# apple/swift-homomorphic-encryption

Hardware: NVIDIA H100
Metric: BFV ct*ct mults/sec at N=8192, 4 coefficient moduli (higher is better)
Workload: dtype u64

## Files before the change

### swift-homomorphic-encryption_b200/csrc/behz.cu

```cuda
#include <cstdlib>

#include "kernels.cuh"

namespace hecuda {

constexpr int kThreads = 128;

static int cols_per_thread() {
    static const int v = [] {
        const char *e = std::getenv("HECUDA_BEHZ_COLS");
        return (e && e[0] == '1') ? 1 : 2;
    }();
    return v;
}

template <int COLS>
struct Cols {
    u64 v[COLS];
};
template <int COLS>
__device__ __forceinline__ Cols<COLS> ldc(const u64 *p) {
    Cols<COLS> r;
    if (COLS == 2) {
        const ulonglong2 t = *reinterpret_cast<const ulonglong2 *>(p);
        r.v[0] = t.x;
        r.v[COLS - 1] = t.y;
    } else {
        r.v[0] = *p;
    }
    return r;
}
template <int COLS>
__device__ __forceinline__ void stc(u64 *p, const u64 (&v)[COLS]) {
    if (COLS == 2) *reinterpret_cast<ulonglong2 *>(p) = make_ulonglong2(v[0], v[COLS - 1]);
    else *p = v[0];
}

template <int L, int COLS>
__global__ void __launch_bounds__(kThreads) lift_kernel(const u64 *__restrict__ in, int polys_in, u64 *__restrict__ ext,
                                                       int ext_polys, int out_poly_offset,
                                                       const __grid_constant__ LiftConsts c, int n, bool q_rows) {
    const int rows_out = q_rows ? 2 * L + 1 : L + 1, aux0 = q_rows ? L : 0;
    const int coeff = (blockIdx.x * kThreads + threadIdx.x) * COLS;
    if (coeff >= n) return;
    const int64_t poly = (int64_t)blockIdx.z * gridDim.y + blockIdx.y;
    const int64_t item = polys_in == 2 ? (poly >> 1) : poly / polys_in;
    const int pin = (int)(poly - item * polys_in);
    const u64 *src = in + poly * L * n + coeff;
    u64 *dst = ext + ((item * ext_polys + out_poly_offset + pin) * rows_out) * n + coeff;
    u64 z[COLS][L];
    u32 acc_mt[COLS];
#pragma unroll
    for (int k = 0; k < COLS; ++k) acc_mt[k] = 0;
#pragma unroll
    for (int i = 0; i < L; ++i) {
        const Cols<COLS> x = ldc<COLS>(src + (int64_t)i * n);
        if (q_rows) stc<COLS>(dst + (int64_t)i * n, x.v);
#pragma unroll
        for (int k = 0; k < COLS; ++k) {
            z[k][i] = shoup_mul(x.v[k], c.in_w[i], c.in_wp[i], c.q[i]);
            acc_mt[k] += (u32)z[k][i] * c.punct_mt[i];
        }
    }
    u32 r[COLS];
    bool neg[COLS];
#pragma unroll
    for (int k = 0; k < COLS; ++k) {
        r[k] = (acc_mt[k] * c.neg_inv_q_mt) & c.mt_mask;
        neg[k] = r[k] >= c.mt_half;
    }
#pragma unroll
    for (int j = 0; j <= L; ++j) {
        u64 o[COLS];
#pragma unroll
        for (int k = 0; k < COLS; ++k) {
            const u64 rc = neg[k] ? (u64)r[k] + c.neg_off[j] : (u64)r[k];
            u128 acc = (u128)rc * c.qr[j];
#pragma unroll
            for (int i = 0; i < L; ++i) mac128(acc, z[k][i], c.mat[j][i]);
            const u64 red = mont_reduce(acc, c.b[j], c.b_ninv[j]);
            o[k] = c.wide_sums ? barrett64(red, c.b[j], c.b_mu1[j]) : csub(red, c.b[j]);
        }
        stc<COLS>(dst + (int64_t)(aux0 + j) * n, o);
    }
}

struct TensorConsts {
    int R;
    u64 p[kMaxRows], ninv[kMaxRows];
};

template <int COLS>
__global__ void __launch_bounds__(kThreads) tensor_kernel(const u64 *__restrict__ ext, u64 *__restrict__ ten,
                                                         const __grid_constant__ TensorConsts c, int n) {
    const int R = c.R;
    const int row = blockIdx.y;
    const int64_t item = blockIdx.z;
    const int coeff = (blockIdx.x * kThreads + threadIdx.x) * COLS;
    if (coeff >= n) return;
    const u64 p = c.p[row], ninv = c.ninv[row];
    const u64 *e = ext + (item * 4 * R + row) * n + coeff;
    const int64_t ps = (int64_t)R * n;
    const Cols<COLS> a0 = ldc<COLS>(e), a1 = ldc<COLS>(e + ps), b0 = ldc<COLS>(e + 2 * ps), b1 = ldc<COLS>(e + 3 * ps);
    u64 *o = ten + (item * 3 * R + row) * n + coeff;
    u64 o0[COLS], o1[COLS], o2[COLS];
#pragma unroll
    for (int k = 0; k < COLS; ++k) {
        o0[k] = csub(mont_reduce((u128)a0.v[k] * b0.v[k], p, ninv), p);
        u128 m = (u128)a0.v[k] * b1.v[k];
        mac128(m, a1.v[k], b0.v[k]);
        o1[k] = csub(mont_reduce(m, p, ninv), p);
        o2[k] = csub(mont_reduce((u128)a1.v[k] * b1.v[k], p, ninv), p);
    }
    stc<COLS>(o, o0);
    stc<COLS>(o + ps, o1);
    stc<COLS>(o + 2 * ps, o2);
}

struct TensorSumConsts {
    int R;
    long long max_pairs;
    u64 p[kMaxRows], ninv[kMaxRows], mu1[kMaxRows], mu_hi[kMaxRows], mu_lo[kMaxRows];
};

__global__ void __launch_bounds__(kThreads) tensor_sum_kernel(const u64 *__restrict__ ext, u64 *__restrict__ ten,
                                                             const __grid_constant__ TensorSumConsts c, int n,
                                                             long long pairs) {
    const int R = c.R;
    const int row = blockIdx.y;
    const int64_t group = blockIdx.z;
    const int coeff = (blockIdx.x * kThreads + threadIdx.x) * 2;
    if (coeff >= n) return;
    const u64 p = c.p[row], ninv = c.ninv[row];
    const int64_t ps = (int64_t)R * n;
    const u64 *e = ext + (group * pairs * 4 * R + row) * n + coeff;
    u128 a0[2] = {0, 0}, a1[2] = {0, 0}, a2[2] = {0, 0};
    long long since = 0;
    for (long long k = 0; k < pairs; ++k, e += 4 * ps) {
        const Cols<2> l0 = ldc<2>(e), l1 = ldc<2>(e + ps), r0 = ldc<2>(e + 2 * ps), r1 = ldc<2>(e + 3 * ps);
#pragma unroll
        for (int j = 0; j < 2; ++j) {
            mac128(a0[j], l0.v[j], r0.v[j]);
            mac128(a1[j], l0.v[j], r1.v[j]);
            mac128(a1[j], l1.v[j], r0.v[j]);
            mac128(a2[j], l1.v[j], r1.v[j]);
        }
        if (++since >= c.max_pairs) {
            since = 0;
#pragma unroll
            for (int j = 0; j < 2; ++j) {
                u128w w0 = {(u64)a0[j], (u64)(a0[j] >> 64)}, w1 = {(u64)a1[j], (u64)(a1[j] >> 64)},
                      w2 = {(u64)a2[j], (u64)(a2[j] >> 64)};
                a0[j] = barrett128(w0, p, c.mu_hi[row], c.mu_lo[row]);
                a1[j] = barrett128(w1, p, c.mu_hi[row], c.mu_lo[row]);
                a2[j] = barrett128(w2, p, c.mu_hi[row], c.mu_lo[row]);
            }
        }
    }
    u64 *o = ten + (group * 3 * R + row) * n + coeff;
    u64 o0[2], o1[2], o2[2];
    const u64 mu1 = c.mu1[row];
#pragma unroll
    for (int j = 0; j < 2; ++j) {
        o0[j] = barrett64(mont_reduce(a0[j], p, ninv), p, mu1);
        o1[j] = barrett64(mont_reduce(a1[j], p, ninv), p, mu1);
        o2[j] = barrett64(mont_reduce(a2[j], p, ninv), p, mu1);
    }
    stc<2>(o, o0);
    stc<2>(o + ps, o1);
    stc<2>(o + 2 * ps, o2);
}

template <int L, int COLS>
__global__ void __launch_bounds__(kThreads) floor_kernel(const u64 *__restrict__ in, u64 *__restrict__ out,
                                                        const __grid_constant__ FloorConsts c, int n) {
    constexpr int R = 2 * L + 1;
    const int coeff = (blockIdx.x * kThreads + threadIdx.x) * COLS;
    if (coeff >= n) return;
    const int64_t poly = (int64_t)blockIdx.z * gridDim.y + blockIdx.y;
    const u64 *src = in + poly * R * n + coeff;
    u64 *dst = out + poly * L * n + coeff;
    u64 y[COLS][L];
#pragma unroll
    for (int i = 0; i < L; ++i) {
        const Cols<COLS> x = ldc<COLS>(src + (int64_t)i * n);
#pragma unroll
        for (int k = 0; k < COLS; ++k) y[k][i] = shoup_mul(x.v[k], c.inq_w[i], c.inq_wp[i], c.q[i]);
    }
    u64 f[COLS][L + 1];
#pragma unroll
    for (int j = 0; j <= L; ++j) {
        const Cols<COLS> xb = ldc<COLS>(src + (int64_t)(L + j) * n);
#pragma unroll
        for (int k = 0; k < COLS; ++k) {
            u128 acc = (u128)xb.v[k] * c.fq[j];
#pragma unroll
            for (int i = 0; i < L; ++i) mac128(acc, y[k][i], c.fmat[j][i]);
            f[k][j] = mont_reduce(acc, c.b[j], c.b_ninv[j]);
        }
    }
    const u64 msk = c.b[L];
    u64 outv[L][COLS];
#pragma unroll
    for (int k = 0; k < COLS; ++k) {
        u64 w[L];
        u128 acc = (u128)f[k][L] * c.a_msk;
#pragma unroll
        for (int i = 0; i < L; ++i) {
            w[i] = shoup_mul(f[k][i], c.inb_w[i], c.inb_wp[i], c.b[i]);
            mac128(acc, w[i], c.amat[i]);
        }
        u64 alpha = mont_reduce(acc, msk, c.b_ninv[L]);
        alpha = c.wide_sums ? barrett64(alpha, msk, c.msk_mu1) : csub(csub(csub(alpha, 4 * msk), 2 * msk), msk);
        const bool exceeds = alpha > (msk >> 1);
        const u64 alpha_c = exceeds ? msk - alpha : alpha;
#pragma unroll
        for (int i = 0; i < L; ++i) {
            u128 o = (u128)alpha_c * (exceeds ? c.b_mod_q[i] : c.neg_b_mod_q[i]);
#pragma unroll
            for (int kk = 0; kk < L; ++kk) mac128(o, w[kk], c.omat[i][kk]);
            outv[i][k] = csub(csub(mont_reduce(o, c.q[i], c.q_ninv[i]), 2 * c.q[i]), c.q[i]);
        }
    }
#pragma unroll
    for (int i = 0; i < L; ++i) stc<COLS>(dst + (int64_t)i * n, outv[i]);
}

__global__ void __launch_bounds__(kThreads) lift_generic_kernel(const u64 *__restrict__ in, int polys_in, u64 *__restrict__ ext,
                                                               int ext_polys, int out_poly_offset,
                                                               const __grid_constant__ LiftConsts c, int n, bool q_rows) {
    const int L = c.L, rows_out = q_rows ? 2 * L + 1 : L + 1, aux0 = q_rows ? L : 0;
    const int coeff = blockIdx.x * kThreads + threadIdx.x;
    if (coeff >= n) return;
    const int64_t poly = (int64_t)blockIdx.z * gridDim.y + blockIdx.y;
    const int64_t item = poly / polys_in;
    const int pin = (int)(poly - item * polys_in);
    const u64 *src = in + poly * L * n + coeff;
    u64 *dst = ext + ((item * ext_polys + out_poly_offset + pin) * rows_out) * n + coeff;
    u64 z[kMaxL];
    u32 acc_mt = 0;
    for (int i = 0; i < L; ++i) {
        const u64 x = src[(int64_t)i * n];
        if (q_rows) dst[(int64_t)i * n] = x;
        z[i] = shoup_mul(x, c.in_w[i], c.in_wp[i], c.q[i]);
        acc_mt += (u32)z[i] * c.punct_mt[i];
    }
    const u32 r = (acc_mt * c.neg_inv_q_mt) & c.mt_mask;
    const bool neg = r >= c.mt_half;
    for (int j = 0; j <= L; ++j) {
        const u64 rc = neg ? (u64)r + c.neg_off[j] : (u64)r;
        u128 acc = (u128)rc * c.qr[j];
        for (int i = 0; i < L; ++i) mac128(acc, z[i], c.mat[j][i]);
        const u64 red = mont_reduce(acc, c.b[j], c.b_ninv[j]);
        dst[(int64_t)(aux0 + j) * n] = c.wide_sums ? barrett64(red, c.b[j], c.b_mu1[j]) : csub(red, c.b[j]);
    }
}

__global__ void __launch_bounds__(kThreads) floor_generic_kernel(const u64 *__restrict__ in, u64 *__restrict__ out,
                                                                const __grid_constant__ FloorConsts c, int n) {
    const int L = c.L, R = 2 * L + 1;
    const int coeff = blockIdx.x * kThreads + threadIdx.x;
    if (coeff >= n) return;
    const int64_t poly = (int64_t)blockIdx.z * gridDim.y + blockIdx.y;
    const u64 *src = in + poly * R * n + coeff;
    u64 *dst = out + poly * L * n + coeff;
    u64 y[kMaxL], f[kMaxL + 1], w[kMaxL];
    for (int i = 0; i < L; ++i) y[i] = shoup_mul(src[(int64_t)i * n], c.inq_w[i], c.inq_wp[i], c.q[i]);
    for (int j = 0; j <= L; ++j) {
        u128 acc = (u128)src[(int64_t)(L + j) * n] * c.fq[j];
        for (int i = 0; i < L; ++i) mac128(acc, y[i], c.fmat[j][i]);
        f[j] = mont_reduce(acc, c.b[j], c.b_ninv[j]);
    }
    const u64 msk = c.b[L];
    u128 acc = (u128)f[L] * c.a_msk;
    for (int i = 0; i < L; ++i) {
        w[i] = shoup_mul(f[i], c.inb_w[i], c.inb_wp[i], c.b[i]);
        mac128(acc, w[i], c.amat[i]);
    }
    u64 alpha = mont_reduce(acc, msk, c.b_ninv[L]);
    alpha = c.wide_sums ? barrett64(alpha, msk, c.msk_mu1) : csub(csub(csub(alpha, 4 * msk), 2 * msk), msk);
    const bool exceeds = alpha > (msk >> 1);
    const u64 alpha_c = exceeds ? msk - alpha : alpha;
    for (int i = 0; i < L; ++i) {
        u128 o = (u128)alpha_c * (exceeds ? c.b_mod_q[i] : c.neg_b_mod_q[i]);
        for (int kk = 0; kk < L; ++kk) mac128(o, w[kk], c.omat[i][kk]);
        dst[(int64_t)i * n] = barrett64(mont_reduce(o, c.q[i], c.q_ninv[i]), c.q[i], c.q_mu1[i]);
    }
}

#define HE_DISPATCH_L(L_, CALL)                                                                                       \
    switch (L_) {                                                                                                     \
        case 1: { constexpr int LL = 1; CALL; } break;                                                                \
        case 2: { constexpr int LL = 2; CALL; } break;                                                                \
        case 3: { constexpr int LL = 3; CALL; } break;                                                                \
        case 4: { constexpr int LL = 4; CALL; } break;                                                                \
        case 5: { constexpr int LL = 5; CALL; } break;                                                                \
        case 6: { constexpr int LL = 6; CALL; } break;                                                                \
        case 7: { constexpr int LL = 7; CALL; } break;                                                                \
        case 8: { constexpr int LL = 8; CALL; } break;                                                                \
        case 9: { constexpr int LL = 9; CALL; } break;                                                                \
        case 10: { constexpr int LL = 10; CALL; } break;                                                              \
        case 11: { constexpr int LL = 11; CALL; } break;                                                              \
        case 12: { constexpr int LL = 12; CALL; } break;                                                              \
        case 13: { constexpr int LL = 13; CALL; } break;                                                              \
        case 14: { constexpr int LL = 14; CALL; } break;                                                              \
        case 15: { constexpr int LL = 15; CALL; } break;                                                              \
        case 16: { constexpr int LL = 16; CALL; } break;                                                              \
        default: return cudaErrorInvalidValue;                                                                        \
    }

static inline dim3 poly_grid(int64_t n, int64_t polys, int cols) {
    const unsigned gx = (unsigned)((n / cols + kThreads - 1) / kThreads);
    const int64_t gy = polys < 32768 ? polys : 32768;
    return dim3(gx ? gx : 1, (unsigned)gy, (unsigned)((polys + gy - 1) / gy));
}

cudaError_t launch_lift(const Context &ctx, const u64 *in, int polys_in, u64 *ext, int ext_polys, int out_poly_offset,
                        int64_t items, cudaStream_t stream, bool reference_base, bool q_rows) {
    const LiftConsts &consts = reference_base ? ctx.lift : ctx.lift_mul;
    int64_t polys = items * polys_in;
    if (polys == 0) return cudaSuccess;
    const int64_t pstride_in = (int64_t)ctx.L * ctx.n;
    while (polys > 0) {
        int64_t slab = polys >= 32768 ? (polys / 32768) * 32768 : polys;
        const int cols = ctx.L > 16 ? 1 : (ctx.n >= 2 ? cols_per_thread() : 1);
        const dim3 grid = poly_grid(ctx.n, slab, cols);
        ++g_kernel_launches;
        if (ctx.L > 16) {
            lift_generic_kernel<<<grid, kThreads, 0, stream>>>(in, polys_in, ext, ext_polys, out_poly_offset, consts, (int)ctx.n, q_rows);
        } else if (cols == 2) {
            HE_DISPATCH_L(ctx.L, (lift_kernel<LL, 2><<<grid, kThreads, 0, stream>>>(in, polys_in, ext, ext_polys,
                                                                                 out_poly_offset, consts, (int)ctx.n, q_rows)));
        } else {
            HE_DISPATCH_L(ctx.L, (lift_kernel<LL, 1><<<grid, kThreads, 0, stream>>>(in, polys_in, ext, ext_polys,
                                                                                 out_poly_offset, consts, (int)ctx.n, q_rows)));
        }
        in += slab * pstride_in;
        ext += (slab / polys_in) * (int64_t)ext_polys * (q_rows ? 2 * ctx.L + 1 : ctx.L + 1) * ctx.n;
        polys -= slab;
    }
    return cudaGetLastError();
}

cudaError_t launch_tensor(const Context &ctx, const u64 *ext, u64 *ten, int64_t items, cudaStream_t stream,
                          bool reference_base) {
    if (items == 0) return cudaSuccess;
    TensorConsts tc;
    tc.R = 2 * ctx.L + 1;
    const NttRowMap map = reference_base ? ctx.map_qbsk() : ctx.map_qaux();
    for (int r = 0; r < tc.R; ++r) {
        tc.p[r] = ctx.slots[map.slot[r]].dev.p;
        tc.ninv[r] = ctx.slots[map.slot[r]].dev.ninv;
    }
    const int cols = ctx.n >= 2 ? cols_per_thread() : 1;
    const unsigned gx = (unsigned)((ctx.n / cols + kThreads - 1) / kThreads);
    for (int64_t done = 0; done < items;) {
        const int64_t chunk = (items - done) > 65535 ? 65535 : (items - done);
        dim3 grid(gx ? gx : 1, (unsigned)tc.R, (unsigned)chunk);
        ++g_kernel_launches;
        if (cols == 2)
            tensor_kernel<2><<<grid, kThreads, 0, stream>>>(ext + done * 4 * tc.R * ctx.n, ten + done * 3 * tc.R * ctx.n, tc,
                                                            (int)ctx.n);
        else
            tensor_kernel<1><<<grid, kThreads, 0, stream>>>(ext + done * 4 * tc.R * ctx.n, ten + done * 3 * tc.R * ctx.n, tc,
                                                            (int)ctx.n);
        done += chunk;
    }
    return cudaGetLastError();
}

cudaError_t launch_tensor_sum(const Context &ctx, const u64 *ext, u64 *ten, int64_t pairs, int64_t groups,
                              cudaStream_t stream, bool reference_base) {
    if (groups == 0) return cudaSuccess;
    if (ctx.n < 2 || pairs < 1) return cudaErrorInvalidValue;
    TensorSumConsts tc;
    tc.R = 2 * ctx.L + 1;
    const NttRowMap map = reference_base ? ctx.map_qbsk() : ctx.map_qaux();
    u64 pmax = 0;
    for (int r = 0; r < tc.R; ++r) {
        const ModSlot &S = ctx.slots[map.slot[r]].dev;
        tc.p[r] = S.p;
        tc.ninv[r] = S.ninv;
        tc.mu1[r] = S.mu1;
        tc.mu_hi[r] = S.mu_hi;
        tc.mu_lo[r] = S.mu_lo;
        pmax = S.p > pmax ? S.p : pmax;
    }
    const u128 per_pair = 2 * (u128)pmax * pmax;
    const u128 cap = (((u128)1) << 127) / per_pair;
    tc.max_pairs = cap < 1 ? 1 : (cap > (u128)0x7fffffffLL ? 0x7fffffffLL : (long long)cap);
    const unsigned gx = (unsigned)((ctx.n / 2 + kThreads - 1) / kThreads);
    for (int64_t done = 0; done < groups;) {
        const int64_t chunk = (groups - done) > 65535 ? 65535 : (groups - done);
        dim3 grid(gx ? gx : 1, (unsigned)tc.R, (unsigned)chunk);
        ++g_kernel_launches;
        tensor_sum_kernel<<<grid, kThreads, 0, stream>>>(ext + done * pairs * 4 * tc.R * ctx.n, ten + done * 3 * tc.R * ctx.n,
                                                         tc, (int)ctx.n, pairs);
        done += chunk;
    }
    return cudaGetLastError();
}

cudaError_t launch_floor(const Context &ctx, const u64 *in, u64 *out, int64_t polys, cudaStream_t stream,
                         bool reference_base) {
    if (polys == 0) return cudaSuccess;
    const FloorConsts &consts = reference_base ? ctx.floor : ctx.floor_mul;
    const int R = 2 * ctx.L + 1;
    while (polys > 0) {
        int64_t slab = polys >= 32768 ? (polys / 32768) * 32768 : polys;
        const int cols = ctx.L > 16 ? 1 : (ctx.n >= 2 ? cols_per_thread() : 1);
        const dim3 grid = poly_grid(ctx.n, slab, cols);
        ++g_kernel_launches;
        if (ctx.L > 16) {
            floor_generic_kernel<<<grid, kThreads, 0, stream>>>(in, out, consts, (int)ctx.n);
        } else if (cols == 2) {
            HE_DISPATCH_L(ctx.L, (floor_kernel<LL, 2><<<grid, kThreads, 0, stream>>>(in, out, consts, (int)ctx.n)));
        } else {
            HE_DISPATCH_L(ctx.L, (floor_kernel<LL, 1><<<grid, kThreads, 0, stream>>>(in, out, consts, (int)ctx.n)));
        }
        in += slab * (int64_t)R * ctx.n;
        out += slab * (int64_t)ctx.L * ctx.n;
        polys -= slab;
    }
    return cudaGetLastError();
}

}
```

### swift-homomorphic-encryption_b200/csrc/context.cu

```cuda
#include "context.hpp"

#include <cuda_runtime.h>

#include <cmath>
#include <cstdlib>
#include <cstring>

#include "hostmath.hpp"
#include "ntt_fast.cuh"

namespace hecuda {
using namespace host;


static void fill_barrett(u64 p, u64 &mu1, u64 &mu_hi, u64 &mu_lo) {
    mu1 = (u64)(((u128)1 << 64) / p);
    u128 mu = (p & (p - 1)) == 0 ? ((u128)1 << (128 - (bit_length(p) - 1))) : (~(u128)0) / p;
    mu_hi = (u64)(mu >> 64);
    mu_lo = (u64)mu;
}

static bool build_slot(HostSlot &hs, u64 p, int64_t n, int logn, u64 t, std::vector<ulonglong2> &tw,
                       std::vector<ulonglong2> &itw, std::string &err) {
    if (!is_prime(p) || (p - 1) % (2 * (u64)n) != 0) {
        err = "invalidNttModulus: " + std::to_string(p) + " is not a prime = 1 mod 2N";
        return false;
    }
    if (p >= (1ull << 62)) {
        err = "invalidModulus: " + std::to_string(p) + " exceeds 2^62 - 1";
        return false;
    }
    ModSlot &d = hs.dev;
    std::memset(&d, 0, sizeof(d));
    d.p = p;
    fill_barrett(p, d.mu1, d.mu_hi, d.mu_lo);
    d.bits = bit_length(p);
    d.s_prod = d.bits - 2;
    d.mu_prod = (u64)(((u128)1 << (d.bits + 62)) / p);
    d.red_shift = d.bits > 12 ? d.bits - 12 : 0;
    d.red_recip = (u32)((((u128)1) << (d.red_shift + 32)) / p);
    const u64 psi = min_primitive_root(2 * (u64)n, p);
    const u64 psi_inv = invmod(psi, p);
    hs.roots.assign(n, 1);
    hs.inv_roots.assign(n, 1);
    u64 pw = 1, ipw = 1;
    for (int64_t i = 0; i < n; ++i) {
        unsigned r = bitrev((unsigned)i, logn);
        hs.roots[r] = pw;
        hs.inv_roots[r] = ipw;
        pw = mulmod(pw, psi, p);
        ipw = mulmod(ipw, psi_inv, p);
    }
    tw.resize(n);
    itw.resize(n);
    for (int64_t i = 0; i < n; ++i) {
        tw[i] = make_ulonglong2(hs.roots[i], shoup_factor(hs.roots[i], p));
        itw[i] = make_ulonglong2(hs.inv_roots[i], shoup_factor(hs.inv_roots[i], p));
    }
    const u64 n_inv = invmod((u64)n % p, p);
    const u64 w1_inv = n > 1 ? hs.inv_roots[1] : 1;
    d.r64 = (u64)(((u128)1 << 64) % p);
    {
        u64 inv = p;
        for (int i = 0; i < 6; ++i) inv *= 2 - p * inv;
        d.ninv = 0 - inv;
    }
    const u64 scalings[3] = {1 % p, mulmod(t % p, d.r64, p), d.r64};
    for (int k = 0; k < 3; ++k) {
        ModSlot::InvScale &sc = d.inv_scale[k];
        sc.c0 = mulmod(n_inv, scalings[k], p);
        sc.c0p = shoup_factor(sc.c0, p);
        sc.c1 = mulmod(sc.c0, w1_inv, p);
        sc.c1p = shoup_factor(sc.c1, p);
    }
    return true;
}

static DivRoundConsts build_divround(const std::vector<u64> &base) {
    DivRoundConsts c;
    std::memset(&c, 0, sizeof(c));
    c.l = (int)base.size();
    c.last = base.back();
    c.half = c.last >> 1;
    for (int i = 0; i + 1 < c.l; ++i) {
        const u64 m = base[i];
        c.m[i] = m;
        c.mu1[i] = (u64)(((u128)1 << 64) / m);
        c.half_mod[i] = c.half % m;
        c.inv_w[i] = invmod(c.last % m, m);
        c.inv_wp[i] = shoup_factor(c.inv_w[i], m);
    }
    return c;
}

Context *Context::create(int64_t n, const u64 *coeff_moduli, int nmod, u64 t, std::string &err, int word_bits) {
    if (word_bits != 64 && word_bits != 32) { err = "invalidEncryptionParameters: word size must be 32 or 64"; return nullptr; }
    for (int i = 0; i < nmod; ++i)
        if (coeff_moduli[i] >> (word_bits - 2)) { err = "invalidModulus: " + std::to_string(coeff_moduli[i]) + " exceeds the maximum of this word size"; return nullptr; }
    if (n < 2 || (n & (n - 1)) || n > (1 << 17)) { err = "invalidDegree: N must be a power of two in [2, 2^17]"; return nullptr; }
    if (n > (1 << fast::kSplitLogN)) { err = "unsupportedHeOperation: polynomial degrees above 2^" + std::to_string(fast::kSplitLogN) + " are not supported by the NTT kernels"; return nullptr; }
    if (nmod < 1) { err = "invalidEncryptionParameters: need at least one coefficient modulus"; return nullptr; }
    if (nmod > kMaxL) { err = "invalidEncryptionParameters: more than " + std::to_string(kMaxL) + " coefficient moduli (EncryptionParameters.swift:148)"; return nullptr; }
    if (t < 2) { err = "invalidEncryptionParameters: plaintext modulus"; return nullptr; }
    for (int i = 0; i < nmod; ++i)
        for (int j = 0; j < i; ++j)
            if (coeff_moduli[i] == coeff_moduli[j]) { err = "coprimeModuli: repeated coefficient modulus"; return nullptr; }

    Context *c = new Context();
    c->n = n;
    c->logn = bit_length((u64)n) - 1;
    c->has_ks = nmod >= 2;
    c->L = c->has_ks ? nmod - 1 : 1;
    c->t = t;
    c->word_bits = word_bits;
    c->mtilde = word_bits == 64 ? (1ull << 32) : (1ull << 16);
    c->gamma = word_bits == 64 ? ((1ull << 62) - 40797) : ((1ull << 30) - 20405);
    const u64 kMTilde = c->mtilde;
    cudaGetDevice(&c->device);
    c->sm_count = 1;
    cudaDeviceGetAttribute(&c->sm_count, cudaDevAttrMultiProcessorCount, c->device);
    const int L = c->L;
    c->q.assign(coeff_moduli, coeff_moduli + L);
    c->q_ks = c->has_ks ? coeff_moduli[L] : 0;
    for (u64 qi : c->q)
        if (t >= qi) { err = "invalidEncryptionParameters: plaintext modulus must be below every coefficient modulus"; delete c; return nullptr; }
    c->bsk = smallest_ntt_primes(word_bits - 3, L + 1, (u64)n);
    if ((int)c->bsk.size() != L + 1) { err = "notEnoughPrimes for Bsk"; delete c; return nullptr; }
    for (u64 b : c->bsk)
        for (int i = 0; i < nmod; ++i)
            if (b == coeff_moduli[i]) { err = "coprimeModuli: coefficient modulus collides with the BEHZ base"; delete c; return nullptr; }

    c->aux = c->bsk;
    {
        const char *env = std::getenv("HECUDA_AUX_BASE");
        const bool want_fast = !(env && std::string(env) == "reference");
        const int widths[2] = {30, 55};
        double log_q = 0;
        for (u64 v : c->q) log_q += std::log2((double)v);
        const double log_n = (double)c->logn, log_t = std::log2((double)t);
        for (int wi = 0; wi < 2 && want_fast && c->aux == c->bsk && word_bits == 64; ++wi) {
            const bool h_primes = fast::kNarrowHEnabled && std::getenv("HECUDA_AUX_H_PRIMES") != nullptr;
            std::vector<u64> cand = (widths[wi] == 55 && h_primes) ? smallest_ntt_primes(55, L + 1 + nmod, 1ull << 31)
                                                                   : smallest_ntt_primes(widths[wi], L + 1 + nmod, (u64)n);
            std::vector<u64> pick;
            for (u64 v : cand) {
                bool used = false;
                for (int i = 0; i < nmod; ++i) used |= coeff_moduli[i] == v;
                if (!used && (int)pick.size() < L + 1) pick.push_back(v);
            }
            double log_aux = 0, log_aux_l = 0;
            for (size_t j = 0; j < pick.size(); ++j) {
                log_aux += std::log2((double)pick[j]);
                if ((int)j < L) log_aux_l += std::log2((double)pick[j]);
            }
            const bool enough = (int)pick.size() == L + 1 && log_aux >= log_q + log_n + 4 &&
                                log_aux_l + std::log2((double)pick.back()) >= log_t + log_n + log_q + 5;
            if (enough) c->aux = pick;
        }
    }
    c->aux_is_reference = c->aux == c->bsk;

    const int nslots = c->aux_is_reference ? 2 * L + 2 : 3 * L + 3;
    c->slots.resize(nslots);
    std::vector<u64> slot_mod(nslots);
    for (int i = 0; i < L; ++i) slot_mod[c->slot_q(i)] = c->q[i];
    for (int j = 0; j <= L; ++j) slot_mod[c->slot_bsk(j)] = c->bsk[j];
    slot_mod[c->slot_ks()] = c->q_ks;
    if (!c->aux_is_reference)
        for (int j = 0; j <= L; ++j) slot_mod[c->slot_aux(j)] = c->aux[j];
    const size_t table_bytes = sizeof(ulonglong2) * (size_t)n;
    const bool fast = c->logn >= fast::kMinLogN && c->logn <= fast::kMaxLogN;
    const bool split = c->logn == fast::kSplitLogN;
    const int half_logn = c->logn - 1;
    const int64_t half_n = n / 2;
    const int threads = (int)((split ? half_n : n) / 16);
    const size_t tr_bytes = (fast || split) ? sizeof(ulonglong2) * (size_t)15 * threads : 0;
    const size_t half_bytes = sizeof(ulonglong2) * (size_t)half_n;
    const size_t slot_bytes = 2 * table_bytes + (split ? 2 * (2 * half_bytes + 2 * tr_bytes) : 2 * tr_bytes);
    if (cudaMalloc(&c->d_pool, slot_bytes * nslots) != cudaSuccess) { err = "cudaMalloc failed for twiddle tables"; delete c; return nullptr; }
    std::vector<ulonglong2> tw, itw, tr(15 * (size_t)threads), itr(15 * (size_t)threads), twh, itwh;
    std::vector<ModSlot> dev_slots(split ? 3 * nslots : nslots);
    c->split_slot_base = split ? nslots : 0;
    for (int s = 0; s < nslots; ++s) {
        if (s == c->slot_ks() && !c->has_ks) {
            std::memset(&c->slots[s].dev, 0, sizeof(ModSlot));
            dev_slots[s] = c->slots[s].dev;
            continue;
        }
        if (!build_slot(c->slots[s], slot_mod[s], n, c->logn, t, tw, itw, err)) { delete c; return nullptr; }
        char *base = (char *)c->d_pool + slot_bytes * s;
        cudaMemcpy(base, tw.data(), table_bytes, cudaMemcpyHostToDevice);
        cudaMemcpy(base + table_bytes, itw.data(), table_bytes, cudaMemcpyHostToDevice);
        c->slots[s].dev.tw = (const ulonglong2 *)base;
        c->slots[s].dev.itw = (const ulonglong2 *)(base + table_bytes);
        if (fast) {
            for (int k = 0; k < 15; ++k)
                for (int tau = 0; tau < threads; ++tau) {
                    tr[(size_t)k * threads + tau] = tw[fast::fwd_last_source(c->logn, k, tau)];
                    itr[(size_t)k * threads + tau] = itw[fast::inv_first_source(c->logn, k, tau)];
                }
            cudaMemcpy(base + 2 * table_bytes, tr.data(), tr_bytes, cudaMemcpyHostToDevice);
            cudaMemcpy(base + 2 * table_bytes + tr_bytes, itr.data(), tr_bytes, cudaMemcpyHostToDevice);
            c->slots[s].dev.tw_t = (const ulonglong2 *)(base + 2 * table_bytes);
            c->slots[s].dev.itw_t = (const ulonglong2 *)(base + 2 * table_bytes + tr_bytes);
        }
        dev_slots[s] = c->slots[s].dev;
        if (split) {
            for (int hh = 0; hh < 2; ++hh) {
                twh.assign(half_n, tw[0]);
                itwh.assign(half_n, itw[0]);
                for (int64_t i = 1; i < half_n; ++i) {
                    const int sp = bit_length((u64)i) - 1;
                    const int64_t src = ((int64_t)(2 + hh) << sp) + (i - ((int64_t)1 << sp));
                    twh[i] = tw[src];
                    itwh[i] = itw[src];
                }
                for (int k = 0; k < 15; ++k)
                    for (int tau = 0; tau < threads; ++tau) {
                        tr[(size_t)k * threads + tau] = twh[fast::fwd_last_source(half_logn, k, tau)];
                        itr[(size_t)k * threads + tau] = itwh[fast::inv_first_source(half_logn, k, tau)];
                    }
                char *hb = base + 2 * table_bytes + hh * (2 * half_bytes + 2 * tr_bytes);
                cudaMemcpy(hb, twh.data(), half_bytes, cudaMemcpyHostToDevice);
                cudaMemcpy(hb + half_bytes, itwh.data(), half_bytes, cudaMemcpyHostToDevice);
                cudaMemcpy(hb + 2 * half_bytes, tr.data(), tr_bytes, cudaMemcpyHostToDevice);
                cudaMemcpy(hb + 2 * half_bytes + tr_bytes, itr.data(), tr_bytes, cudaMemcpyHostToDevice);
                ModSlot v = c->slots[s].dev;
                v.tw = (const ulonglong2 *)hb;
                v.itw = (const ulonglong2 *)(hb + half_bytes);
                v.tw_t = (const ulonglong2 *)(hb + 2 * half_bytes);
                v.itw_t = (const ulonglong2 *)(hb + 2 * half_bytes + tr_bytes);
                dev_slots[nslots + 2 * s + hh] = v;
            }
        }
    }
    if (cudaMalloc(&c->d_slots, sizeof(ModSlot) * dev_slots.size()) != cudaSuccess) { err = "cudaMalloc failed"; delete c; return nullptr; }
    cudaMemcpy(c->d_slots, dev_slots.data(), sizeof(ModSlot) * dev_slots.size(), cudaMemcpyHostToDevice);

    const u64 *Q = c->q.data();
    auto build_behz = [&](const std::vector<u64> &base, bool reference_base, LiftConsts &lf, FloorConsts &fl) {
    const u64 *BSK = base.data();
    const u64 msk = base[L];
    auto slot_of = [&](int j) { return reference_base ? c->slot_bsk(j) : c->slot_aux(j); };
    std::memset(&lf, 0, sizeof(lf));
    lf.L = L;
    {
        const u64 q_mod_mt = prod_mod(Q, L, kMTilde);
        lf.neg_inv_q_mt = (u32)((kMTilde - invmod(q_mod_mt, kMTilde)) % kMTilde);
    }
    for (int i = 0; i < L; ++i) {
        const u64 qi = Q[i];
        lf.q[i] = qi;
        const u64 inv_punct = invmod(punctured_mod(Q, L, i, qi), qi);
        lf.in_w[i] = mulmod(kMTilde % qi, inv_punct, qi);
        lf.in_wp[i] = shoup_factor(lf.in_w[i], qi);
        lf.punct_mt[i] = (u32)punctured_mod(Q, L, i, kMTilde);
    }
    lf.mt_mask = (u32)(kMTilde - 1);
    lf.mt_half = (u32)(kMTilde >> 1);
    for (int j = 0; j <= L; ++j) lf.neg_off[j] = ((kMTilde + BSK[j] - 1) / BSK[j]) * BSK[j] - kMTilde;
    for (int j = 0; j <= L; ++j) {
        const u64 bj = BSK[j];
        lf.b[j] = bj;
        lf.b_ninv[j] = c->slots[slot_of(j)].dev.ninv;
        const u64 r64 = c->slots[slot_of(j)].dev.r64;
        const u64 mt_inv = mulmod(invmod(kMTilde % bj, bj), r64, bj);
        for (int i = 0; i < L; ++i) lf.mat[j][i] = mulmod(punctured_mod(Q, L, i, bj), mt_inv, bj);
        lf.qr[j] = mulmod(prod_mod(Q, L, bj), mt_inv, bj);
    }
    std::memset(&fl, 0, sizeof(fl));
    fl.L = L;
    const u64 b_mod_msk = prod_mod(BSK, L, msk);
    const u64 r64_msk = c->slots[slot_of(L)].dev.r64;
    const u64 b_inv_msk = mulmod(invmod(b_mod_msk, msk), r64_msk, msk);
    fl.a_msk = (msk - b_inv_msk) % msk;
    for (int i = 0; i < L; ++i) {
        const u64 qi = Q[i];
        fl.q[i] = qi;
        fl.q_ninv[i] = c->slots[c->slot_q(i)].dev.ninv;
        fl.q_mu1[i] = c->slots[c->slot_q(i)].dev.mu1;
        const u64 r64 = c->slots[c->slot_q(i)].dev.r64;
        fl.inq_w[i] = invmod(punctured_mod(Q, L, i, qi), qi);
        fl.inq_wp[i] = shoup_factor(fl.inq_w[i], qi);
        for (int k = 0; k < L; ++k) fl.omat[i][k] = mulmod(punctured_mod(BSK, L, k, qi), r64, qi);
        fl.b_mod_q[i] = mulmod(prod_mod(BSK, L, qi), r64, qi);
        fl.neg_b_mod_q[i] = (qi - fl.b_mod_q[i]) % qi;
    }
    for (int j = 0; j <= L; ++j) {
        const u64 bj = BSK[j];
        fl.b[j] = bj;
        fl.b_ninv[j] = c->slots[slot_of(j)].dev.ninv;
        const u64 q_inv = mulmod(invmod(prod_mod(Q, L, bj), bj), c->slots[slot_of(j)].dev.r64, bj);
        fl.fq[j] = q_inv;
        for (int i = 0; i < L; ++i) {
            const u64 v = mulmod(punctured_mod(Q, L, i, bj), q_inv, bj);
            fl.fmat[j][i] = (bj - v) % bj;
        }
    }
    for (int k = 0; k < L; ++k) {
        const u64 bk = BSK[k];
        fl.inb_w[k] = invmod(punctured_mod(BSK, L, k, bk), bk);
        fl.inb_wp[k] = shoup_factor(fl.inb_w[k], bk);
        fl.amat[k] = mulmod(punctured_mod(BSK, L, k, msk), b_inv_msk, msk);
    }
    };
    build_behz(c->bsk, true, c->lift, c->floor);
    if (c->aux_is_reference) {
        c->lift_mul = c->lift;
        c->floor_mul = c->floor;
    } else {
        build_behz(c->aux, false, c->lift_mul, c->floor_mul);
    }

    auto check_ranges = [&](const std::vector<u64> &base, LiftConsts &lf, FloorConsts &fl) -> bool {
        u64 qmax = 0, bmax = 0;
        for (u64 v : c->q) qmax = v > qmax ? v : qmax;
        for (u64 v : base) bmax = v > bmax ? v : bmax;
        const double worst = std::log2((double)(L + 2)) + std::log2((double)qmax) + std::log2((double)bmax);
        if (worst >= 127.0) return false;
        const bool wide = (u128)bmax + (u128)L * qmax >= ((u128)1 << 64);
        lf.wide_sums = fl.wide_sums = wide ? 1 : 0;
        for (int j = 0; j <= L; ++j) lf.b_mu1[j] = (u64)(((u128)1 << 64) / base[j]);
        fl.msk_mu1 = (u64)(((u128)1 << 64) / base[L]);
        return true;
    };
    if (!check_ranges(c->bsk, c->lift, c->floor) || !check_ranges(c->aux, c->lift_mul, c->floor_mul)) {
        err = "unsupportedHeOperation: " + std::to_string(L) + " ciphertext moduli of this size overflow the 128-bit lazy sums";
        delete c;
        return nullptr;
    }

    {
        u64 mmax = c->q_ks;
        for (u64 v : c->q) mmax = v > mmax ? v : mmax;
        if (std::log2((double)L) + 2 * std::log2((double)mmax) >= 128.0) {
            err = "unsupportedHeOperation: " + std::to_string(L) + " moduli of this size overflow the key-switching accumulator";
            delete c;
            return nullptr;
        }
    }

    c->ks_divround.resize(L + 1);
    c->ms_divround.resize(L + 1);
    for (int l = 1; l <= L; ++l) {
        std::vector<u64> base(c->q.begin(), c->q.begin() + l);
        if (l >= 2) c->ms_divround[l] = build_divround(base);
        if (!c->has_ks) continue;
        base.push_back(c->q_ks);
        c->ks_divround[l] = build_divround(base);
    }
    cudaError_t e = cudaDeviceSynchronize();
    if (e != cudaSuccess) { err = std::string("CUDA error during context setup: ") + cudaGetErrorString(e); delete c; return nullptr; }
    return c;
}

Context::~Context() {
    if (d_pool) cudaFree(d_pool);
    if (d_slots) cudaFree(d_slots);
}

NttRowMap Context::map_q(int rows) const {
    NttRowMap m;
    std::memset(&m, 0, sizeof(m));
    m.rows_per_poly = rows;
    m.group = 1;
    m.src_mod = 0;
    m.src_poly_stride = 0;
    for (int r = 0; r < rows; ++r) m.slot[r] = (unsigned char)slot_q(r);
    return m;
}
NttRowMap Context::map_qbsk() const {
    NttRowMap m;
    std::memset(&m, 0, sizeof(m));
    m.rows_per_poly = 2 * L + 1;
    m.group = 1;
    m.src_mod = 0;
    m.src_poly_stride = 0;
    for (int r = 0; r < L; ++r) m.slot[r] = (unsigned char)slot_q(r);
    for (int j = 0; j <= L; ++j) m.slot[L + j] = (unsigned char)slot_bsk(j);
    return m;
}
NttRowMap Context::map_qaux() const {
    NttRowMap m = map_qbsk();
    if (!aux_is_reference)
        for (int j = 0; j <= L; ++j) m.slot[L + j] = (unsigned char)slot_aux(j);
    return m;
}
NttRowMap Context::map_ks(int l) const {
    NttRowMap m;
    std::memset(&m, 0, sizeof(m));
    m.rows_per_poly = l + 1;
    m.group = 1;
    m.src_mod = 0;
    m.src_poly_stride = 0;
    for (int r = 0; r < l; ++r) m.slot[r] = (unsigned char)slot_q(r);
    m.slot[l] = (unsigned char)slot_ks();
    return m;
}
NttRowMap Context::map_single(int slot) const {
    NttRowMap m;
    std::memset(&m, 0, sizeof(m));
    m.rows_per_poly = 1;
    m.group = 1;
    m.src_mod = 0;
    m.src_poly_stride = 0;
    m.slot[0] = (unsigned char)slot;
    return m;
}
NttRowMap Context::map_ks_digits(int l, long long target_poly_stride) const {
    NttRowMap m = map_ks(l);
    m.rows_per_poly = (l + 1) * l;
    m.group = l;
    m.src_mod = l;
    m.src_poly_stride = target_poly_stride;
    for (int j = 0; j < l; ++j) m.src_slot[j] = (unsigned char)slot_q(j);
    return m;
}
int Context::find_slot(u64 modulus) const {
    for (size_t s = 0; s < slots.size(); ++s)
        if (slots[s].dev.p == modulus) return (int)s;
    return -1;
}

}
```

### swift-homomorphic-encryption_b200/csrc/context.hpp

```cpp
#pragma once
#include <cstdint>
#include <string>
#include <vector>

#include "modarith.cuh"

namespace hecuda {

constexpr int kMaxL = 32;
constexpr int kMaxSlots = 3 * kMaxL + 3;
constexpr int kMaxRows = 2 * kMaxL + 1;

struct ModSlot {
    u64 p;
    u64 mu1;
    u64 mu_hi, mu_lo;
    u64 mu_prod;
    int s_prod;
    int bits;
    int red_shift;
    u32 red_recip;
    u64 ninv;
    u64 r64;
    struct InvScale { u64 c0, c0p, c1, c1p; } inv_scale[3];
    const ulonglong2 *tw;
    const ulonglong2 *itw;
    const ulonglong2 *tw_t;
    const ulonglong2 *itw_t;
};

enum { kScalePlain = 0, kScaleTMont = 1, kScaleMont = 2 };

struct NttRowMap {
    int rows_per_poly;
    int group;
    unsigned char slot[kMaxRows + 1];
    int src_mod;
    long long src_poly_stride;
    unsigned char src_slot[kMaxRows + 1];
};

struct LiftConsts {
    int L;
    int wide_sums;
    u64 b_mu1[kMaxL + 1];
    u64 q[kMaxL];
    u64 in_w[kMaxL], in_wp[kMaxL];
    u32 punct_mt[kMaxL];
    u32 neg_inv_q_mt;
    u32 mt_mask, mt_half;
    u64 neg_off[kMaxL + 1];
    u64 b[kMaxL + 1], b_ninv[kMaxL + 1];
    u64 mat[kMaxL + 1][kMaxL];
    u64 qr[kMaxL + 1];
};

struct FloorConsts {
    int L;
    int wide_sums;
    u64 msk_mu1;
    u64 q[kMaxL], q_ninv[kMaxL], q_mu1[kMaxL];
    u64 inq_w[kMaxL], inq_wp[kMaxL];
    u64 b[kMaxL + 1], b_ninv[kMaxL + 1];
    u64 fq[kMaxL + 1];
    u64 fmat[kMaxL + 1][kMaxL];
    u64 inb_w[kMaxL], inb_wp[kMaxL];
    u64 amat[kMaxL];
    u64 a_msk;
    u64 omat[kMaxL][kMaxL];
    u64 b_mod_q[kMaxL], neg_b_mod_q[kMaxL];
};

struct DivRoundConsts {
    int l;
    u64 m[kMaxL + 1], mu1[kMaxL + 1];
    u64 last, half;
    u64 half_mod[kMaxL + 1];
    u64 inv_w[kMaxL + 1], inv_wp[kMaxL + 1];
};

struct HostSlot {
    ModSlot dev;
    std::vector<u64> roots, inv_roots;
};

class Context {
   public:
    static Context *create(int64_t n, const u64 *coeff_moduli, int nmod, u64 t, std::string &err, int word_bits = 64);
    ~Context();

    int64_t n;
    int logn;
    int word_bits = 64;
    u64 mtilde = 1ull << 32;
    u64 gamma = (1ull << 62) - 40797;
    int L;
    u64 t;
    int device;
    int sm_count;
    std::vector<u64> q;
    u64 q_ks;
    bool has_ks = true;
    std::vector<u64> bsk;
    std::vector<u64> aux;
    bool aux_is_reference = true;
    std::vector<HostSlot> slots;
    ModSlot *d_slots = nullptr;
    int split_slot_base = 0;
    LiftConsts lift;
    FloorConsts floor;
    LiftConsts lift_mul;
    FloorConsts floor_mul;
    std::vector<DivRoundConsts> ks_divround;
    std::vector<DivRoundConsts> ms_divround;
    void *d_pool = nullptr;

    int slot_q(int i) const { return i; }
    int slot_bsk(int j) const { return L + j; }
    int slot_ks() const { return 2 * L + 1; }
    int slot_aux(int j) const { return aux_is_reference ? slot_bsk(j) : 2 * L + 2 + j; }
    NttRowMap map_q(int rows) const;
    NttRowMap map_qbsk() const;
    NttRowMap map_qaux() const;
    NttRowMap map_ks(int l) const;
    NttRowMap map_single(int slot) const;
    NttRowMap map_ks_digits(int l, long long target_poly_stride) const;
    int find_slot(u64 modulus) const;
};

}
```

### swift-homomorphic-encryption_b200/csrc/modarith.cuh

```cuda
#pragma once
#include <cstdint>

#if defined(__CUDACC__)
#define HE_HD __host__ __device__ __forceinline__
#define HE_D __device__ __forceinline__
#else
#define HE_HD inline
#define HE_D inline
#endif

namespace hecuda {

typedef unsigned long long u64;
typedef unsigned int u32;

HE_HD u64 mulhi64(u64 a, u64 b) {
#if defined(__CUDA_ARCH__)
    return __umul64hi(a, b);
#else
    return (u64)(((unsigned __int128)a * b) >> 64);
#endif
}

HE_HD u64 csub(u64 x, u64 p) { return x >= p ? x - p : x; }
HE_HD u64 add_mod(u64 a, u64 b, u64 p) { return csub(a + b, p); }
HE_HD u64 sub_mod(u64 a, u64 b, u64 p) { return csub(a + p - b, p); }

HE_HD u64 shoup_lazy(u64 x, u64 w, u64 wp, u64 p) {
    u64 q = mulhi64(x, wp);
    return x * w - q * p;
}
HE_HD u64 shoup_mul(u64 x, u64 w, u64 wp, u64 p) { return csub(shoup_lazy(x, w, wp, p), p); }

HE_HD u64 barrett64(u64 x, u64 p, u64 mu1) {
    u64 q = mulhi64(x, mu1);
    return csub(x - q * p, p);
}

struct u128w {
    u64 lo, hi;
};
HE_HD u128w mul_wide(u64 a, u64 b) {
    u128w r;
    r.lo = a * b;
    r.hi = mulhi64(a, b);
    return r;
}
HE_HD void mac_wide(u128w &acc, u64 a, u64 b) {
    u64 lo = a * b;
    u64 hi = mulhi64(a, b);
    acc.lo += lo;
    acc.hi += hi + (acc.lo < lo ? 1ull : 0ull);
}

HE_HD u64 barrett128(u128w x, u64 p, u64 mu_hi, u64 mu_lo) {
    u64 ll_hi = mulhi64(x.lo, mu_lo);
    u64 lh_lo = x.lo * mu_hi, lh_hi = mulhi64(x.lo, mu_hi);
    u64 hl_lo = x.hi * mu_lo, hl_hi = mulhi64(x.hi, mu_lo);
    u64 hh_lo = x.hi * mu_hi;
    u64 mid = ll_hi + lh_lo;
    u64 c1 = mid < ll_hi ? 1ull : 0ull;
    u64 mid2 = mid + hl_lo;
    u64 c2 = mid2 < mid ? 1ull : 0ull;
    u64 q = hh_lo + lh_hi + hl_hi + c1 + c2;
    return csub(x.lo - q * p, p);
}

typedef unsigned __int128 u128;
HE_HD void mac128(u128 &acc, u64 a, u64 b) { acc += (u128)a * b; }
HE_HD u64 mont_reduce(u128 acc, u64 p, u64 ninv) {
    const u64 lo = (u64)acc, hi = (u64)(acc >> 64);
    const u64 m = lo * ninv;
    return hi + mulhi64(m, p) + (lo != 0 ? 1ull : 0ull);
}

HE_HD u64 barrett_prod(u128w x, u64 p, u64 mu, int s) {
    u64 xs = (x.lo >> s) | (x.hi << (64 - s));
    u64 q = mulhi64(xs, mu);
    u64 r = x.lo - q * p;
    r = csub(r, 4 * p);
    r = csub(r, 2 * p);
    return csub(r, p);
}

}
```

### swift-homomorphic-encryption_b200/csrc/ntt_fast.cu

```cuda
#include <cuda.h>

#include <mutex>

#include <algorithm>
#include <cstdlib>
#include "kernels.cuh"
#include "ntt_fast.cuh"

namespace hecuda {
using namespace fast;

constexpr int kMaxRowList = 2 * (kMaxL + 1) * kMaxL;
struct RowList {
    int rows_per_poly;
    int count;
    unsigned short row[kMaxRowList];
    unsigned short slot[kMaxRowList];
    unsigned char flags[kMaxRowList];
    unsigned short src_row[kMaxRowList];
    long long src_poly_stride;
};

__device__ __forceinline__ u32 smem_u32(const void *p) { return (u32)__cvta_generic_to_shared(p); }
__device__ __forceinline__ void mbar_init(u64 *bar, int count) {
    asm volatile("mbarrier.init.shared::cta.b64 [%0], %1;" ::"r"(smem_u32(bar)), "r"(count) : "memory");
    asm volatile("fence.mbarrier_init.release.cluster;" ::: "memory");
}
__device__ __forceinline__ void mbar_arrive_expect_tx(u64 *bar, u32 bytes) {
    asm volatile("mbarrier.arrive.expect_tx.shared::cta.b64 _, [%0], %1;" ::"r"(smem_u32(bar)), "r"(bytes) : "memory");
}
__device__ __forceinline__ void mbar_wait(u64 *bar, u32 parity) {
    asm volatile(
        "{\n\t.reg .pred done;\n\t"
        "WAIT_%=:\n\t"
        "mbarrier.try_wait.parity.shared::cta.b64 done, [%0], %1;\n\t"
        "@!done bra WAIT_%=;\n\t}" ::"r"(smem_u32(bar)),
        "r"(parity)
        : "memory");
}
__device__ __forceinline__ void tma_load_1d(void *smem_dst, const void *gmem_src, u32 bytes, u64 *bar) {
    asm volatile("cp.async.bulk.shared::cluster.global.mbarrier::complete_tx::bytes [%0], [%1], %2, [%3];" ::"r"(smem_u32(smem_dst)),
                 "l"(gmem_src), "r"(bytes), "r"(smem_u32(bar))
                 : "memory");
}
__device__ __forceinline__ void tma_load_box(void *smem_dst, const CUtensorMap *map, int line, u64 *bar) {
    asm volatile("cp.async.bulk.tensor.2d.shared::cluster.global.tile.mbarrier::complete_tx::bytes [%0], [%1, {%2, %3}], [%4];" ::"r"(
                     smem_u32(smem_dst)),
                 "l"(map), "r"(0), "r"(line), "r"(smem_u32(bar))
                 : "memory");
}
__device__ __forceinline__ void tma_store_box(const CUtensorMap *map, int line, const void *smem_src) {
    asm volatile("cp.async.bulk.tensor.2d.global.shared::cta.tile.bulk_group [%0, {%1, %2}], [%3];" ::"l"(map), "r"(0), "r"(line),
                 "r"(smem_u32(smem_src))
                 : "memory");
}
__device__ __forceinline__ void tma_prefetch_box(const CUtensorMap *map, int line) {
    asm volatile("cp.async.bulk.prefetch.tensor.2d.L2.global.tile [%0, {%1, %2}];" ::"l"(map), "r"(0), "r"(line) : "memory");
}
__device__ __forceinline__ void tma_commit() { asm volatile("cp.async.bulk.commit_group;" ::: "memory"); }
template <int PENDING>
__device__ __forceinline__ void tma_store_wait_read() { asm volatile("cp.async.bulk.wait_group.read %0;" ::"n"(PENDING) : "memory"); }
__device__ __forceinline__ void tma_store_wait_all() { asm volatile("cp.async.bulk.wait_group 0;" ::: "memory"); }
__device__ __forceinline__ void fence_proxy_async_smem() { asm volatile("fence.proxy.async.shared::cta;" ::: "memory"); }

template <int LOGN, int CLS, int K>
__device__ __forceinline__ void fwd_row_pass(u64 (&x)[16], u64 *sm, int tau, const RowMod &m, bool reduce_in) {
    constexpr int P = plan_passes(LOGN), C = fwd_c(LOGN, K), LB = fwd_lb(LOGN, K);
    load_smem<LOGN, LB, C>(x, sm, tau);
    if (K == 0 && reduce_in) {
#pragma unroll
        for (int r = 0; r < 16; ++r) x[r] = barrett64(x[r], 0 - m.np, m.slot->mu1);
    }
    fwd_pass<LOGN, LB, C, CLS>(x, tau, m);
    if (K == P - 1) fwd_finish<CLS>(x, m);
    store_smem<LOGN, LB, C>(x, sm, tau);
}
template <int LOGN, int CLS>
__device__ __forceinline__ void fwd_row(u64 *sm, int tau, const RowMod &m, bool reduce_in) {
    constexpr int P = plan_passes(LOGN);
    u64 x[16];
    fwd_row_pass<LOGN, CLS, 0>(x, sm, tau, m, reduce_in);
    __syncthreads();
    fwd_row_pass<LOGN, CLS, 1>(x, sm, tau, m, false);
    __syncthreads();
    if (P == 4) {
        fwd_row_pass<LOGN, CLS, (P == 4 ? 2 : 1)>(x, sm, tau, m, false);
        __syncthreads();
    }
    fwd_row_pass<LOGN, CLS, P - 1>(x, sm, tau, m, false);
}

template <int LOGN, int CLS, int K>
__device__ __forceinline__ void inv_row_pass(u64 (&x)[16], u64 *sm, int tau, const RowMod &m) {
    constexpr int C = inv_c(LOGN, K), LB = inv_lb(LOGN, K);
    load_smem<LOGN, LB, C>(x, sm, tau);
    if (narrow_like(CLS) && K > 0 && inv_reduce_at(LOGN, K)) inv_reduce(x, m);
    inv_pass<LOGN, LB, C, CLS, inv_bound_in(LOGN, K)>(x, tau, m);
    if (K == plan_passes(LOGN) - 1 && m.partial) {
        if (CLS == kSmall) {
#pragma unroll
            for (int r = 0; r < 16; ++r) x[r] = csub32((u32)x[r], (u32)(0 - m.np));
        } else {
            reduce_small16(x, m);
        }
    }
    store_smem<LOGN, LB, C>(x, sm, tau);
}
template <int LOGN, int CLS>
__device__ __forceinline__ void inv_row(u64 *sm, int tau, const RowMod &m) {
    constexpr int P = plan_passes(LOGN);
    u64 x[16];
    inv_row_pass<LOGN, CLS, 0>(x, sm, tau, m);
    __syncthreads();
    inv_row_pass<LOGN, CLS, 1>(x, sm, tau, m);
    __syncthreads();
    if (P == 4) {
        inv_row_pass<LOGN, CLS, (P == 4 ? 2 : 1)>(x, sm, tau, m);
        __syncthreads();
    }
    inv_row_pass<LOGN, CLS, P - 1>(x, sm, tau, m);
}

HE_HD constexpr int ntt_row_buffers(int logn) { return logn == 13 ? 2 : 1; }

template <int LOGN>
constexpr size_t ntt_smem_bytes() {
    constexpr int B = ntt_row_buffers(LOGN);
    return sizeof(u64) * B * ((size_t)1 << LOGN) + sizeof(ulonglong2) * ((size_t)1 << (LOGN - 4)) + sizeof(u64) * (B + 1);
}

constexpr int ntt_min_ctas(int logn) { return logn == 13 ? 1 : 1024 / ((1 << logn) / 16); }

template <int LOGN, bool INVERSE>
__global__ void __launch_bounds__((1 << LOGN) / 16, ntt_min_ctas(LOGN))
    ntt_rows_kernel(const __grid_constant__ CUtensorMap map_in, const __grid_constant__ CUtensorMap map_out,
                    const ModSlot *__restrict__ slots, const __grid_constant__ RowList rl, const int polys,
                    const int scale_mode, const int debug_flags) {
    extern __shared__ __align__(1024) u64 smem[];
    constexpr int kLines = (1 << LOGN) / kLineWords;
    constexpr int kBoxes = kLines > kBoxLines ? kLines / kBoxLines : 1;
    constexpr int kLinesPerBox = kLines / kBoxes;
    constexpr u32 kRowBytes = (u32)sizeof(u64) << LOGN, kTwBytes = (u32)sizeof(ulonglong2) << (LOGN - 4);
    constexpr int B = ntt_row_buffers(LOGN), AHEAD = B > 1 ? 1 : 0;
    ulonglong2 *tw_cache = reinterpret_cast<ulonglong2 *>(smem + B * (1 << LOGN));
    u64 *bar_row = reinterpret_cast<u64 *>(tw_cache + (1 << (LOGN - 4)));
    u64 *bar_tw = bar_row + B;
    const int tau = threadIdx.x;
    const int tasks = polys * rl.count;
    auto in_line = [&](int t) {
        const int w = t / polys, p = t - w * polys;
        const int64_t word = INVERSE ? ((int64_t)p * rl.rows_per_poly + rl.row[w]) << LOGN
                                     : (int64_t)p * rl.src_poly_stride + ((int64_t)rl.src_row[w] << LOGN);
        return (int)(word >> 4);
    };
    auto load_row = [&](int t, int buf) {
        mbar_arrive_expect_tx(&bar_row[buf], kRowBytes);
        const int line = in_line(t);
        u64 *dst = smem + buf * (1 << LOGN);
#pragma unroll
        for (int b = 0; b < kBoxes; ++b) tma_load_box(dst + b * kLinesPerBox * kLineWords, &map_in, line + b * kLinesPerBox, &bar_row[buf]);
    };
    if (tau == 0) {
        if (smem_u32(smem) & 1023) __trap();
#pragma unroll
        for (int b = 0; b < B; ++b) mbar_init(&bar_row[b], 1);
        mbar_init(bar_tw, 1);
        if (AHEAD && (int)blockIdx.x < tasks) load_row(blockIdx.x, 0);
    }
    __syncthreads();
    u32 phase_row = 0, phase_tw = 0;
    int cached_slot = -1;
    int buf = 0;
    for (int task = blockIdx.x; task < tasks; task += gridDim.x) {
        const int which = task / polys;
        const int poly = task - which * polys;
        const int flags = rl.flags[which];
        const int slot = rl.slot[which];
        const ModSlot &S = slots[slot];
        u64 *sm = smem + buf * (1 << LOGN);
        const int64_t out_word = ((int64_t)poly * rl.rows_per_poly + rl.row[which]) << LOGN;
        const bool new_slot = slot != cached_slot;
        cached_slot = slot;
        if (tau == 0) {
            if (new_slot) {
                mbar_arrive_expect_tx(bar_tw, kTwBytes);
                tma_load_1d(tw_cache, INVERSE ? S.itw : S.tw, kTwBytes, bar_tw);
            }
            const int fill = task + AHEAD * gridDim.x;
            if (fill < tasks) {
                tma_store_wait_read<B - 1 - AHEAD>();
                load_row(fill, (buf + AHEAD) % B);
            }
            const int next = fill + gridDim.x;
            if (next < tasks && !(debug_flags & 1)) {
                const int line = in_line(next);
#pragma unroll
                for (int b = 0; b < kBoxes; ++b) tma_prefetch_box(&map_in, line + b * kLinesPerBox);
            }
        }
        const int cls = flags & 7;
        RowMod m;
        m.np = 0 - S.p;
        m.kp = (cls == kWide || cls == kSmall) ? 2 * S.p : 4 * S.p;
        m.tw = nullptr;
        m.tw_s = smem_u32(tw_cache);
        m.slot = &S;
        m.scale_mode = INVERSE ? scale_mode : -1;
        m.partial = INVERSE && (flags & 16) != 0;
        if (new_slot) {
            mbar_wait(bar_tw, phase_tw);
            phase_tw ^= 1;
        }
        mbar_wait(&bar_row[buf], (phase_row >> buf) & 1);
        phase_row ^= 1u << buf;
        if (debug_flags & 4) {
        } else
#ifndef HE_EXPERIMENT_ONLY_CLASS
        if (INVERSE) {
            if (kNarrowHEnabled && cls == kNarrowH) inv_row<LOGN, kNarrowHEnabled ? kNarrowH : kNarrow>(sm, tau, m);
            else if (cls == kNarrow) inv_row<LOGN, kNarrow>(sm, tau, m);
            else if (cls == kSmall) inv_row<LOGN, kSmall>(sm, tau, m);
            else if (cls == kMid) inv_row<LOGN, kMid>(sm, tau, m);
            else inv_row<LOGN, kWide>(sm, tau, m);
        } else {
            const bool reduce_in = (flags & 8) != 0;
            if (kNarrowHEnabled && cls == kNarrowH) fwd_row<LOGN, kNarrowHEnabled ? kNarrowH : kNarrow>(sm, tau, m, reduce_in);
            else if (cls == kNarrow) fwd_row<LOGN, kNarrow>(sm, tau, m, reduce_in);
            else if (cls == kSmall) fwd_row<LOGN, kSmall>(sm, tau, m, reduce_in);
            else if (cls == kMid) fwd_row<LOGN, kMid>(sm, tau, m, reduce_in);
            else fwd_row<LOGN, kWide>(sm, tau, m, reduce_in);
        }
#else
        if (INVERSE) inv_row<LOGN, HE_EXPERIMENT_ONLY_CLASS>(sm, tau, m);
        else fwd_row<LOGN, HE_EXPERIMENT_ONLY_CLASS>(sm, tau, m, (flags & 8) != 0);
#endif
        fence_proxy_async_smem();
        __syncthreads();
        if (tau == 0 && !(debug_flags & 2)) {
            const int line = (int)(out_word >> 4);
#pragma unroll
            for (int b = 0; b < kBoxes; ++b) tma_store_box(&map_out, line + b * kLinesPerBox, sm + b * kLinesPerBox * kLineWords);
            tma_commit();
        }
        buf = buf + 1 == B ? 0 : buf + 1;
    }
    if (tau == 0) tma_store_wait_all();
}

__device__ __forceinline__ u32 cluster_ctarank() {
    u32 r;
    asm("mov.u32 %0, %%cluster_ctarank;" : "=r"(r));
    return r;
}
__device__ __forceinline__ int cluster_id_x() {
    u32 r;
    asm("mov.u32 %0, %%clusterid.x;" : "=r"(r));
    return (int)r;
}
__device__ __forceinline__ int cluster_count_x() {
    u32 r;
    asm("mov.u32 %0, %%nclusterid.x;" : "=r"(r));
    return (int)r;
}
__device__ __forceinline__ void cluster_arrive() { asm volatile("barrier.cluster.arrive.release.aligned;" ::: "memory"); }
__device__ __forceinline__ void cluster_wait() { asm volatile("barrier.cluster.wait.acquire.aligned;" ::: "memory"); }
__device__ __forceinline__ void cluster_arrive_relaxed() { asm volatile("barrier.cluster.arrive.relaxed.aligned;" ::: "memory"); }
__device__ __forceinline__ u32 cluster_map(u32 addr, u32 rank) {
    u32 r;
    asm volatile("mapa.shared::cluster.u32 %0, %1, %2;" : "=r"(r) : "r"(addr), "r"(rank));
    return r;
}
__device__ __forceinline__ ulonglong2 ld_cluster_v2(u32 addr) {
    ulonglong2 v;
    asm volatile("ld.shared::cluster.v2.u64 {%0, %1}, [%2];" : "=l"(v.x), "=l"(v.y) : "r"(addr) : "memory");
    return v;
}
__device__ __forceinline__ u64 mont_product(u64 a, u64 b, u64 p, u64 ninv) { return csub(mont_reduce((u128)a * b, p, ninv), p); }

template <int LOGN>
constexpr size_t ntt_tensor_smem_bytes() {
    return sizeof(u64) * 2 * ((size_t)1 << LOGN) + sizeof(ulonglong2) * ((size_t)1 << (LOGN - 4)) + sizeof(u64) * 3;
}

template <int LOGN>
__global__ void __launch_bounds__((1 << LOGN) / 16, 1)
    ntt_forward_tensor_kernel(const __grid_constant__ CUtensorMap map_lhs, const __grid_constant__ CUtensorMap map_rhs,
                              const __grid_constant__ CUtensorMap map_ext, u64 *__restrict__ ten,
                              const ModSlot *__restrict__ slots, const __grid_constant__ RowList rl, const int items,
                              const int L) {
    extern __shared__ __align__(1024) u64 smem[];
    constexpr int N = 1 << LOGN, T = N / 16;
    constexpr int kBoxes = N / kLineWords / kBoxLines;
    constexpr u32 kRowBytes = (u32)sizeof(u64) << LOGN, kTwBytes = (u32)sizeof(ulonglong2) << (LOGN - 4);
    static_assert(kBoxes >= 1, "one row is at least one box");
    ulonglong2 *tw_cache = reinterpret_cast<ulonglong2 *>(smem + 2 * N);
    u64 *bar_row = reinterpret_cast<u64 *>(tw_cache + N / 16);
    u64 *bar_tw = bar_row + 2;
    const int tau = threadIdx.x;
    const u32 rank = cluster_ctarank();
    const int first = cluster_id_x(), stride = cluster_count_x();
    const int R = rl.rows_per_poly;
    const int tasks = items * rl.count;
    auto load_row = [&](int t, int j) {
        const int w = t / items, item = t - w * items, r = rl.row[w];
        const CUtensorMap *map;
        int64_t word;
        if (r < L) {
            map = j ? &map_rhs : &map_lhs;
            word = ((int64_t)(2 * item + (int)rank) * L + r) << LOGN;
        } else {
            map = &map_ext;
            word = ((int64_t)(4 * item + 2 * j + (int)rank) * (L + 1) + r - L) << LOGN;
        }
        const int line = (int)(word >> 4);
        mbar_arrive_expect_tx(&bar_row[j], kRowBytes);
#pragma unroll
        for (int b = 0; b < kBoxes; ++b) tma_load_box(smem + j * N + b * kBoxLines * kLineWords, map, line + b * kBoxLines, &bar_row[j]);
    };
    if (tau == 0) {
        if (smem_u32(smem) & 1023) __trap();
        mbar_init(&bar_row[0], 1);
        mbar_init(&bar_row[1], 1);
        mbar_init(bar_tw, 1);
    }
    cluster_arrive();
    cluster_wait();
    u32 phase_row = 0, phase_tw = 0;
    int cached_slot = -1;
    for (int task = first; task < tasks; task += stride) {
        if (task != first) cluster_wait();
        const int which = task / items;
        const int item = task - which * items;
        const int slot = rl.slot[which], r = rl.row[which], cls = rl.flags[which] & 7;
        const ModSlot &S = slots[slot];
        const bool new_slot = slot != cached_slot;
        cached_slot = slot;
        if (tau == 0) {
            if (new_slot) {
                mbar_arrive_expect_tx(bar_tw, kTwBytes);
                tma_load_1d(tw_cache, S.tw, kTwBytes, bar_tw);
            }
            load_row(task, 0);
            load_row(task, 1);
        }
        RowMod m;
        m.np = 0 - S.p;
        m.kp = (cls == kWide || cls == kSmall) ? 2 * S.p : 4 * S.p;
        m.tw = nullptr;
        m.tw_s = smem_u32(tw_cache);
        m.slot = &S;
        m.scale_mode = -1;
        m.partial = false;
        if (new_slot) {
            mbar_wait(bar_tw, phase_tw);
            phase_tw ^= 1;
        }
#pragma unroll
        for (int j = 0; j < 2; ++j) {
            mbar_wait(&bar_row[j], phase_row);
            u64 *sm = smem + j * N;
            if (kNarrowHEnabled && cls == kNarrowH) fwd_row<LOGN, kNarrowHEnabled ? kNarrowH : kNarrow>(sm, tau, m, false);
            else if (cls == kNarrow) fwd_row<LOGN, kNarrow>(sm, tau, m, false);
            else if (cls == kSmall) fwd_row<LOGN, kSmall>(sm, tau, m, false);
            else if (cls == kMid) fwd_row<LOGN, kMid>(sm, tau, m, false);
            else fwd_row<LOGN, kWide>(sm, tau, m, false);
        }
        phase_row ^= 1;
        __syncthreads();
        cluster_arrive();
        const u64 p = S.p, ninv = S.ninv;
        const u64 *x = smem, *y = smem + N;
        const int64_t comp = (int64_t)R * N;
        u64 *out = ten + ((int64_t)3 * item * R + r) * N;
        u64 *own = out + (rank ? 2 * comp : 0);
#pragma unroll 4
        for (int w = 2 * tau; w < N; w += 2 * T) {
            const ulonglong2 a = *reinterpret_cast<const ulonglong2 *>(x + w), b = *reinterpret_cast<const ulonglong2 *>(y + w);
            *reinterpret_cast<ulonglong2 *>(own + smem_phys(w)) = make_ulonglong2(mont_product(a.x, b.x, p, ninv), mont_product(a.y, b.y, p, ninv));
        }
        cluster_wait();
        const u32 px = cluster_map(smem_u32(x), rank ^ 1), py = cluster_map(smem_u32(y), rank ^ 1);
#pragma unroll 4
        for (int w = (int)rank * (N / 2) + 2 * tau; w < ((int)rank + 1) * (N / 2); w += 2 * T) {
            const ulonglong2 a = *reinterpret_cast<const ulonglong2 *>(x + w), b = *reinterpret_cast<const ulonglong2 *>(y + w);
            const ulonglong2 A = ld_cluster_v2(px + 8u * w), Bv = ld_cluster_v2(py + 8u * w);
            u128 m0 = (u128)a.x * Bv.x, m1 = (u128)a.y * Bv.y;
            mac128(m0, A.x, b.x);
            mac128(m1, A.y, b.y);
            *reinterpret_cast<ulonglong2 *>(out + comp + smem_phys(w)) =
                make_ulonglong2(csub(mont_reduce(m0, p, ninv), p), csub(mont_reduce(m1, p, ninv), p));
        }
        fence_proxy_async_smem();
        cluster_arrive_relaxed();
    }
    if (first < tasks) cluster_wait();
}

static void build_row_list(const Context &ctx, const NttRowMap &map, bool inverse, RowList &rl) {
    rl.rows_per_poly = map.rows_per_poly;
    rl.count = 0;
    rl.src_poly_stride = map.src_mod ? map.src_poly_stride : (long long)map.rows_per_poly * ctx.n;
    static const int order[5] = {kWide, kMid, kNarrow, kNarrowH, kSmall};
    for (int oi = 0; oi < 5; ++oi) {
        const int cls = order[oi];
        for (int r = 0; r < map.rows_per_poly; ++r) {
            const int slot = map.slot[r / map.group];
            if (class_of_modulus(ctx.slots[slot].dev.p, ctx.slots[slot].dev.bits) != cls) continue;
            const int i = rl.count++;
            rl.row[i] = (unsigned short)r;
            rl.slot[i] = (unsigned short)slot;
            rl.src_row[i] = (unsigned short)(map.src_mod && !inverse ? r % map.src_mod : r);
            int flags = cls;
            if (map.src_mod && !inverse) {
                const u64 p = ctx.slots[slot].dev.p, src_p = ctx.slots[map.src_slot[r % map.src_mod]].dev.p;
                const u64 room = narrow_like(cls) ? 2u : cls == kMid ? 8u : cls == kSmall ? 1u : 4u;
                if (src_p > p && (src_p - 1) / p >= room) flags |= 8;
            }
            rl.flags[i] = (unsigned char)flags;
        }
    }
}

typedef CUresult (*EncodeTiledFn)(CUtensorMap *, CUtensorMapDataType, cuuint32_t, void *, const cuuint64_t *, const cuuint64_t *,
                                  const cuuint32_t *, const cuuint32_t *, CUtensorMapInterleave, CUtensorMapSwizzle,
                                  CUtensorMapL2promotion, CUtensorMapFloatOOBfill);
static EncodeTiledFn encode_tiled() {
    static EncodeTiledFn fn = [] {
        void *p = nullptr;
        cudaDriverEntryPointQueryResult q;
        if (cudaGetDriverEntryPoint("cuTensorMapEncodeTiled", &p, cudaEnableDefault, &q) != cudaSuccess || q != cudaDriverEntryPointSuccess)
            p = nullptr;
        return (EncodeTiledFn)p;
    }();
    return fn;
}
static bool make_line_map(CUtensorMap *map, const u64 *base, int logn) {
    EncodeTiledFn enc = encode_tiled();
    if (!enc || (reinterpret_cast<uintptr_t>(base) & 15)) return false;
    const int lines = (1 << logn) / kLineWords;
    const cuuint64_t dims[2] = {kLineWords, (cuuint64_t)1 << 31};
    const cuuint64_t strides[1] = {kLineWords * sizeof(u64)};
    const cuuint32_t box[2] = {kLineWords, (cuuint32_t)(lines > kBoxLines ? kBoxLines : lines)};
    const cuuint32_t elem_strides[2] = {1, 1};
    return enc(map, CU_TENSOR_MAP_DATA_TYPE_UINT64, 2, const_cast<u64 *>(base), dims, strides, box, elem_strides,
               CU_TENSOR_MAP_INTERLEAVE_NONE, CU_TENSOR_MAP_SWIZZLE_128B, CU_TENSOR_MAP_L2_PROMOTION_L2_128B,
               CU_TENSOR_MAP_FLOAT_OOB_FILL_NONE) == CUDA_SUCCESS;
}

template <int LOGN, bool INVERSE>
static cudaError_t launch_logn(const Context &ctx, const NttRowMap &map, const u64 *in, u64 *out, int64_t rows,
                               int scale_mode, cudaStream_t stream) {
    if (rows % map.rows_per_poly) return cudaErrorInvalidValue;
    if (rows == 0) return cudaSuccess;
    if (rows > 0x7fffffffLL) return cudaErrorInvalidValue;
    RowList rl;
    build_row_list(ctx, map, INVERSE, rl);
    if (rl.src_poly_stride % kLineWords) return cudaErrorInvalidValue;
    CUtensorMap map_in, map_out;
    if (!make_line_map(&map_in, in, LOGN) || !make_line_map(&map_out, out, LOGN)) return cudaErrorInvalidValue;
    const int polys = (int)(rows / map.rows_per_poly);
    constexpr int threads = (1 << LOGN) / 16;
    constexpr size_t smem = ntt_smem_bytes<LOGN>();
    auto k = ntt_rows_kernel<LOGN, INVERSE>;
    static int ctas_per_sm[64] = {0};
    static std::mutex mu;
    int per_sm;
    {
        std::lock_guard<std::mutex> lock(mu);
        int &c = ctas_per_sm[ctx.device & 63];
        if (c == 0) {
            cudaError_t e;
            if ((e = cudaFuncSetAttribute(k, cudaFuncAttributeMaxDynamicSharedMemorySize, (int)smem)) != cudaSuccess) return e;
            int n = 0;
            if ((e = cudaOccupancyMaxActiveBlocksPerMultiprocessor(&n, k, threads, smem)) != cudaSuccess) return e;
            if (n < 1) return cudaErrorInvalidConfiguration;
            c = n;
        }
        per_sm = c;
    }
    const int64_t grid = std::min<int64_t>(rows, (int64_t)ctx.sm_count * per_sm);
    ++g_kernel_launches;
    static const int debug_flags = [] {
        const char *env = std::getenv("HECUDA_NTT_DEBUG");
        return env ? std::atoi(env) : 0;
    }();
    k<<<(unsigned)grid, threads, smem, stream>>>(map_in, map_out, ctx.d_slots, rl, polys, scale_mode, debug_flags);
    return cudaGetLastError();
}

struct SplitRows {
    int rows_per_poly, count;
    unsigned short row[kMaxRowList];
    unsigned short src_row[kMaxRowList], slot[kMaxRowList];
    unsigned char reduce_in[kMaxRowList];
    long long src_poly_stride;
};
__global__ void __launch_bounds__(256) ntt_split_forward_kernel(const u64 *__restrict__ in, u64 *__restrict__ out,
                                                               const ModSlot *__restrict__ slots,
                                                               const __grid_constant__ SplitRows sr, int polys, int logn) {
    const int64_t n = (int64_t)1 << logn, half = n >> 1;
    const int which = blockIdx.y;
    const int64_t poly = blockIdx.z;
    const int64_t i = ((int64_t)blockIdx.x * blockDim.x + threadIdx.x) * 2;
    if (i >= half) return;
    const ModSlot &S = slots[sr.slot[which]];
    const u64 p = S.p;
    const ulonglong2 w = S.tw[1];
    const u64 *src = in + poly * sr.src_poly_stride + ((int64_t)sr.src_row[which] << logn) + i;
    u64 *dst = out + (((poly * sr.rows_per_poly) + sr.row[which]) << logn) + i;
    ulonglong2 x = *reinterpret_cast<const ulonglong2 *>(src), y = *reinterpret_cast<const ulonglong2 *>(src + half);
    if (sr.reduce_in[which]) {
        x.x = barrett64(x.x, p, S.mu1), x.y = barrett64(x.y, p, S.mu1);
        y.x = barrett64(y.x, p, S.mu1), y.y = barrett64(y.y, p, S.mu1);
    }
    const u64 v0 = shoup_mul(y.x, w.x, w.y, p), v1 = shoup_mul(y.y, w.x, w.y, p);
    *reinterpret_cast<ulonglong2 *>(dst) = make_ulonglong2(add_mod(x.x, v0, p), add_mod(x.y, v1, p));
    *reinterpret_cast<ulonglong2 *>(dst + half) = make_ulonglong2(sub_mod(x.x, v0, p), sub_mod(x.y, v1, p));
}
__global__ void __launch_bounds__(256) ntt_merge_inverse_kernel(u64 *__restrict__ data, const ModSlot *__restrict__ slots,
                                                               const __grid_constant__ SplitRows sr, int polys, int logn,
                                                               int scale_mode) {
    const int64_t n = (int64_t)1 << logn, half = n >> 1;
    const int which = blockIdx.y;
    const int64_t poly = blockIdx.z;
    const int64_t i = ((int64_t)blockIdx.x * blockDim.x + threadIdx.x) * 2;
    if (i >= half) return;
    const ModSlot &S = slots[sr.slot[which]];
    const u64 p = S.p;
    const ModSlot::InvScale sc = S.inv_scale[scale_mode];
    u64 *row = data + (((poly * sr.rows_per_poly) + sr.row[which]) << logn) + i;
    const ulonglong2 x = *reinterpret_cast<const ulonglong2 *>(row), y = *reinterpret_cast<const ulonglong2 *>(row + half);
    *reinterpret_cast<ulonglong2 *>(row) =
        make_ulonglong2(shoup_mul(x.x + y.x, sc.c0, sc.c0p, p), shoup_mul(x.y + y.y, sc.c0, sc.c0p, p));
    *reinterpret_cast<ulonglong2 *>(row + half) =
        make_ulonglong2(shoup_mul(x.x - y.x + p, sc.c1, sc.c1p, p), shoup_mul(x.y - y.y + p, sc.c1, sc.c1p, p));
}

template <bool INVERSE>
static cudaError_t launch_split(const Context &ctx, const NttRowMap &map, const u64 *in, u64 *out, int64_t rows, int scale_mode,
                                cudaStream_t stream) {
    constexpr int LOGN = kMaxLogN;
    if (rows % map.rows_per_poly) return cudaErrorInvalidValue;
    if (rows == 0) return cudaSuccess;
    if (rows * 2 > 0x7fffffffLL || 2 * map.rows_per_poly > kMaxRowList) return cudaErrorInvalidValue;
    const int polys = (int)(rows / map.rows_per_poly);
    RowList full;
    build_row_list(ctx, map, INVERSE, full);
    SplitRows sr;
    sr.rows_per_poly = full.rows_per_poly;
    sr.count = full.count;
    sr.src_poly_stride = full.src_poly_stride;
    RowList rl;
    rl.rows_per_poly = 2 * full.rows_per_poly;
    rl.count = 2 * full.count;
    rl.src_poly_stride = (long long)rl.rows_per_poly << LOGN;
    for (int i = 0; i < full.count; ++i) {
        sr.row[i] = full.row[i];
        sr.slot[i] = full.slot[i];
        sr.src_row[i] = full.src_row[i];
        sr.reduce_in[i] = (unsigned char)((map.src_mod && !INVERSE) ? 1 : 0);
        for (int hh = 0; hh < 2; ++hh) {
            const int j = 2 * i + hh;
            rl.row[j] = (unsigned short)(2 * full.row[i] + hh);
            rl.src_row[j] = rl.row[j];
            rl.slot[j] = (unsigned short)(ctx.split_slot_base + 2 * full.slot[i] + hh);
            rl.flags[j] = (unsigned char)((full.flags[i] & 7) | (INVERSE ? 16 : 0));
        }
    }
    const dim3 egrid((unsigned)((ctx.n / 4 + 255) / 256), (unsigned)full.count, (unsigned)polys);
    if (!INVERSE) {
        ++g_kernel_launches;
        ntt_split_forward_kernel<<<egrid, 256, 0, stream>>>(in, out, ctx.d_slots, sr, polys, ctx.logn);
        cudaError_t e = cudaGetLastError();
        if (e != cudaSuccess) return e;
        in = out;
    }
    CUtensorMap map_in, map_out;
    if (!make_line_map(&map_in, in, LOGN) || !make_line_map(&map_out, out, LOGN)) return cudaErrorInvalidValue;
    {
        constexpr int threads = (1 << LOGN) / 16;
        constexpr size_t smem = ntt_smem_bytes<LOGN>();
        auto k = ntt_rows_kernel<LOGN, INVERSE>;
        cudaError_t e;
        if ((e = cudaFuncSetAttribute(k, cudaFuncAttributeMaxDynamicSharedMemorySize, (int)smem)) != cudaSuccess) return e;
        int per_sm = 0;
        if ((e = cudaOccupancyMaxActiveBlocksPerMultiprocessor(&per_sm, k, threads, smem)) != cudaSuccess) return e;
        if (per_sm < 1) return cudaErrorInvalidConfiguration;
        const int64_t grid = std::min<int64_t>(2 * rows, (int64_t)ctx.sm_count * per_sm);
        ++g_kernel_launches;
        k<<<(unsigned)grid, threads, smem, stream>>>(map_in, map_out, ctx.d_slots, rl, polys, scale_mode, 0);
        if ((e = cudaGetLastError()) != cudaSuccess) return e;
    }
    if (INVERSE) {
        ++g_kernel_launches;
        ntt_merge_inverse_kernel<<<egrid, 256, 0, stream>>>(out, ctx.d_slots, sr, polys, ctx.logn, scale_mode);
        return cudaGetLastError();
    }
    return cudaSuccess;
}

bool ntt_fast_supported(const Context &ctx) { return ctx.logn >= kMinLogN && ctx.logn <= kSplitLogN; }

template <bool INVERSE>
static cudaError_t launch_fast(const Context &ctx, const NttRowMap &map, const u64 *in, u64 *out, int64_t rows,
                               int scale_mode, cudaStream_t stream) {
    switch (ctx.logn) {
        case 10: return launch_logn<10, INVERSE>(ctx, map, in, out, rows, scale_mode, stream);
        case 11: return launch_logn<11, INVERSE>(ctx, map, in, out, rows, scale_mode, stream);
        case 12: return launch_logn<12, INVERSE>(ctx, map, in, out, rows, scale_mode, stream);
        case 13: return launch_logn<13, INVERSE>(ctx, map, in, out, rows, scale_mode, stream);
        case 14: return launch_logn<14, INVERSE>(ctx, map, in, out, rows, scale_mode, stream);
        case 15: return launch_split<INVERSE>(ctx, map, in, out, rows, scale_mode, stream);
        default: return cudaErrorInvalidValue;
    }
}

cudaError_t launch_ntt_forward_fast(const Context &ctx, const NttRowMap &map, const u64 *in, u64 *out, int64_t rows,
                                    cudaStream_t stream) {
    return launch_fast<false>(ctx, map, in, out, rows, 0, stream);
}
cudaError_t launch_ntt_inverse_fast(const Context &ctx, const NttRowMap &map, const u64 *in, u64 *out, int64_t rows,
                                    int scale_mode, cudaStream_t stream) {
    return launch_fast<true>(ctx, map, in, out, rows, scale_mode, stream);
}

cudaError_t launch_ntt_forward_tensor(const Context &ctx, const NttRowMap &map, const u64 *lhs, const u64 *rhs,
                                      const u64 *ext, u64 *ten, int64_t items, cudaStream_t stream) {
    constexpr int LOGN = 13;
    if (ctx.logn != LOGN) return cudaErrorInvalidValue;
    if (items == 0) return cudaSuccess;
    if (items * 4 * map.rows_per_poly * (ctx.n / kLineWords) > 0x7fffffffLL) return cudaErrorInvalidValue;
    RowList rl;
    build_row_list(ctx, map, false, rl);
    CUtensorMap map_lhs, map_rhs, map_ext;
    if (!make_line_map(&map_lhs, lhs, LOGN) || !make_line_map(&map_rhs, rhs, LOGN) || !make_line_map(&map_ext, ext, LOGN))
        return cudaErrorInvalidValue;
    constexpr int threads = (1 << LOGN) / 16;
    constexpr size_t smem = ntt_tensor_smem_bytes<LOGN>();
    auto k = ntt_forward_tensor_kernel<LOGN>;
    cudaLaunchAttribute attr[1];
    attr[0].id = cudaLaunchAttributeClusterDimension;
    attr[0].val.clusterDim.x = 2;
    attr[0].val.clusterDim.y = 1;
    attr[0].val.clusterDim.z = 1;
    cudaLaunchConfig_t cfg = {};
    cfg.blockDim = dim3(threads);
    cfg.dynamicSmemBytes = smem;
    cfg.stream = stream;
    cfg.attrs = attr;
    cfg.numAttrs = 1;
    static int clusters_per_device[64] = {0};
    static std::mutex mu;
    int clusters;
    {
        std::lock_guard<std::mutex> lock(mu);
        int &c = clusters_per_device[ctx.device & 63];
        if (c == 0) {
            cudaError_t e;
            if ((e = cudaFuncSetAttribute(k, cudaFuncAttributeMaxDynamicSharedMemorySize, (int)smem)) != cudaSuccess) return e;
            cfg.gridDim = dim3(2 * ctx.sm_count);
            int n = 0;
            if ((e = cudaOccupancyMaxActiveClusters(&n, k, &cfg)) != cudaSuccess) return e;
            if (n < 1) return cudaErrorInvalidConfiguration;
            c = n;
        }
        clusters = c;
    }
    const int64_t tasks = items * rl.count;
    cfg.gridDim = dim3((unsigned)(2 * std::min<int64_t>(tasks, clusters)));
    ++g_kernel_launches;
    cudaError_t e = cudaLaunchKernelEx(&cfg, k, map_lhs, map_rhs, map_ext, ten, (const ModSlot *)ctx.d_slots, rl, (int)items, ctx.L);
    return e != cudaSuccess ? e : cudaGetLastError();
}

}
```

### swift-homomorphic-encryption_b200/csrc/ntt_fast.cuh

```cuda
#pragma once
#include "context.hpp"
#include "modarith.cuh"

namespace hecuda {
namespace fast {

constexpr int kMinLogN = 10, kMaxLogN = 14;
constexpr int kSplitLogN = 15;
constexpr int kNarrowBits = 55;
constexpr int kMidBits = 61;
constexpr int kSmallBits = 30;
enum { kNarrow = 0, kMid = 1, kWide = 2, kSmall = 3, kNarrowH = 4 };
HE_HD constexpr int class_of_bits(int bits) {
    return bits <= kSmallBits ? kSmall : bits <= kNarrowBits ? kNarrow : bits <= kMidBits ? kMid : kWide;
}
#if defined(HE_NTT_NARROW_H)
constexpr bool kNarrowHEnabled = true;
#else
constexpr bool kNarrowHEnabled = false;
#endif
HE_HD constexpr int class_of_modulus(u64 p, int bits) {
    return (kNarrowHEnabled && class_of_bits(bits) == kNarrow && (u32)p == 1u) ? kNarrowH : class_of_bits(bits);
}
HE_HD constexpr bool narrow_like(int cls) { return cls == kNarrow || cls == kNarrowH; }

HE_HD constexpr int plan_passes(int logn) { return logn <= 12 ? 3 : 4; }
HE_HD constexpr int plan_c(int logn, int k) {
    return logn == 10   ? (k == 2 ? 4 : 3)
           : logn == 11 ? (k == 1 ? 3 : 4)
           : logn == 12 ? 4
           : logn == 13 ? (k == 3 ? 4 : 3)
                        : (k == 0 || k == 3 ? 4 : 3);
}
HE_HD constexpr int fwd_c(int logn, int k) { return plan_c(logn, k); }
HE_HD constexpr int fwd_lb(int logn, int k) {
    int s0 = 0;
    for (int i = 0; i < k; ++i) s0 += plan_c(logn, i);
    return logn - s0 - plan_c(logn, k);
}
HE_HD constexpr int inv_c(int logn, int k) { return plan_c(logn, plan_passes(logn) - 1 - k); }
HE_HD constexpr int inv_lb(int logn, int k) {
    int u0 = 0;
    for (int i = 0; i < k; ++i) u0 += inv_c(logn, i);
    return u0;
}
HE_HD constexpr int pass_e(int lb, int c) { return lb == 0 ? 0 : 4 - c; }

HE_HD constexpr int inv_stage_bound(int b) { return 2 * b > 4 ? 2 * b : 4; }
HE_HD constexpr int inv_bound_after(int b, int stages) {
    for (int i = 0; i < stages; ++i) b = inv_stage_bound(b);
    return b;
}
HE_HD constexpr bool inv_pass_fits(int b, int stages) {
    for (int i = 0; i < stages; ++i) {
        if (b > 256) return false;
        b = inv_stage_bound(b);
    }
    return true;
}
HE_HD constexpr bool inv_reduce_at(int logn, int k) {
    int b = 1;
    bool red = false;
    for (int i = 0; i <= k; ++i) {
        const int c = inv_c(logn, i);
        red = !inv_pass_fits(b, c);
        if (red) b = 1;
        b = inv_bound_after(b, c);
    }
    return red;
}
HE_HD constexpr int inv_bound_in(int logn, int k) {
    int b = 1;
    for (int i = 0; i <= k; ++i) {
        const int c = inv_c(logn, i);
        if (!inv_pass_fits(b, c)) b = 1;
        if (i < k) b = inv_bound_after(b, c);
    }
    return b;
}

HE_HD constexpr int smem_phys(int e) { return e ^ (((e >> 4) & 7) << 1); }
HE_HD constexpr int smem_words(int logn) { return 1 << logn; }
constexpr int kLineWords = 16;
constexpr int kBoxLines = 256;

HE_HD ulonglong2 ld_tw(const ulonglong2 *p) {
#if defined(__CUDA_ARCH__)
    return __ldg(p);
#else
    return *p;
#endif
}

template <int LOGN, int LB, int C>
HE_HD int elem_index(int tau, int r) {
    constexpr int E = pass_e(LB, C);
    const int lo = tau & ((1 << (LB - E)) - 1), hi = tau >> (LB - E);
    return (hi << (LB + C)) | ((r >> E) << LB) | (lo << E) | (r & ((1 << E) - 1));
}
template <int LB, int C>
HE_HD constexpr int reg_offset(int r) {
    return ((r >> pass_e(LB, C)) << LB) | (r & ((1 << pass_e(LB, C)) - 1));
}
template <int LB, int C>
HE_HD constexpr bool pass_vec() { return pass_e(LB, C) >= 1 || LB == 0; }

template <int LB, int C>
HE_HD int reg_word(int base_phys, int r) {
    constexpr int kSwizzled = 0x7e;
    const int off = reg_offset<LB, C>(r);
    return (off & kSwizzled) ? (base_phys ^ smem_phys(off)) : (base_phys + off);
}

template <int LOGN, int LB, int C>
HE_HD void load_smem(u64 (&x)[16], const u64 *sm, int tau) {
    const int b = smem_phys(elem_index<LOGN, LB, C>(tau, 0));
    if (pass_vec<LB, C>()) {
#pragma unroll
        for (int r = 0; r < 16; r += 2) {
            const ulonglong2 v = *reinterpret_cast<const ulonglong2 *>(sm + reg_word<LB, C>(b, r));
            x[r] = v.x;
            x[r + 1] = v.y;
        }
    } else {
#pragma unroll
        for (int r = 0; r < 16; ++r) x[r] = sm[reg_word<LB, C>(b, r)];
    }
}
template <int LOGN, int LB, int C>
HE_HD void store_smem(const u64 (&x)[16], u64 *sm, int tau) {
    const int b = smem_phys(elem_index<LOGN, LB, C>(tau, 0));
    if (pass_vec<LB, C>()) {
#pragma unroll
        for (int r = 0; r < 16; r += 2)
            *reinterpret_cast<ulonglong2 *>(sm + reg_word<LB, C>(b, r)) = make_ulonglong2(x[r], x[r + 1]);
    } else {
#pragma unroll
        for (int r = 0; r < 16; ++r) sm[reg_word<LB, C>(b, r)] = x[r];
    }
}

struct RowMod {
    u64 np;
    u64 kp;
    const ulonglong2 *tw;
    unsigned tw_s;
    const ModSlot *slot;
    int scale_mode;
    bool partial;
    HE_HD const ulonglong2 *tw_t() const { return scale_mode < 0 ? slot->tw_t : slot->itw_t; }
};
HE_HD ulonglong2 ld_tw_cached(const RowMod &m, int index) {
#if defined(__CUDA_ARCH__)
    ulonglong2 v;
    asm volatile("ld.shared.v2.u64 {%0, %1}, [%2];" : "=l"(v.x), "=l"(v.y) : "r"(m.tw_s + (unsigned)index * 16u));
    return v;
#else
    return m.tw[index];
#endif
}
HE_HD u64 ld_u64(const u64 *p) {
#if defined(__CUDA_ARCH__)
    return __ldg(p);
#else
    return *p;
#endif
}

HE_HD u64 pack64(u32 lo, u32 hi) {
#if defined(__CUDA_ARCH__)
    u64 v;
    asm("mov.b64 %0, {%1, %2};" : "=l"(v) : "r"(lo), "r"(hi));
    return v;
#else
    return ((u64)hi << 32) | lo;
#endif
}
HE_HD void unpack64(u64 v, u32 &lo, u32 &hi) {
#if defined(__CUDA_ARCH__)
    asm("mov.b64 {%0, %1}, %2;" : "=r"(lo), "=r"(hi) : "l"(v));
#else
    lo = (u32)v;
    hi = (u32)(v >> 32);
#endif
}
HE_HD u64 mul_wide_u32(u32 a, u32 b) {
#if defined(__CUDA_ARCH__)
    u64 d;
    asm("mul.wide.u32 %0, %1, %2;" : "=l"(d) : "r"(a), "r"(b));
    return d;
#else
    return (u64)a * b;
#endif
}
HE_HD u64 mad_wide_u32(u32 a, u32 b, u64 c) {
#if defined(__CUDA_ARCH__)
    u64 d;
    asm("mad.wide.u32 %0, %1, %2, %3;" : "=l"(d) : "r"(a), "r"(b), "l"(c));
    return d;
#else
    return (u64)a * b + c;
#endif
}
HE_HD u32 mul_hi_u32(u32 a, u32 b) {
#if defined(__CUDA_ARCH__)
    return __umulhi(a, b);
#else
    return (u32)(((u64)a * b) >> 32);
#endif
}

HE_HD u64 shoup4(u64 y, u64 w, u64 wp, u64 np) {
#if defined(__CUDA_ARCH__)
    u64 v;
    asm volatile("{\n\t"
        ".reg .u32 y0, y1, w0, w1, p0, p1, n0, n1, a1, b1, q0, q1, v0, v1, z;\n\t"
        ".reg .u64 A, B, Q, V;\n\t"
        "mov.b64 {y0, y1}, %1;\n\t"
        "mov.b64 {w0, w1}, %2;\n\t"
        "mov.b64 {p0, p1}, %3;\n\t"
        "mov.b64 {n0, n1}, %4;\n\t"
        "mul.hi.u32 a1, y1, p0;\n\t"
        "mul.hi.u32 b1, y0, p1;\n\t"
        "mov.u32 z, 0;\n\t"
        "mov.b64 A, {a1, z};\n\t"
        "mov.b64 B, {b1, z};\n\t"
        "mad.wide.u32 Q, y1, p1, A;\n\t"
        "add.u64 Q, Q, B;\n\t"
        "mov.b64 {q0, q1}, Q;\n\t"
        "mul.wide.u32 V, y0, w0;\n\t"
        "mad.wide.u32 V, q0, n0, V;\n\t"
        "mov.b64 {v0, v1}, V;\n\t"
        "mad.lo.u32 v1, y1, w0, v1;\n\t"
        "mad.lo.u32 v1, y0, w1, v1;\n\t"
        "mad.lo.u32 v1, q1, n0, v1;\n\t"
        "mad.lo.u32 v1, q0, n1, v1;\n\t"
        "mov.b64 %0, {v0, v1};\n\t}"
        : "=l"(v)
        : "l"(y), "l"(w), "l"(wp), "l"(np));
    return v;
#else
    const u32 y0 = (u32)y, y1 = (u32)(y >> 32), wp0 = (u32)wp, wp1 = (u32)(wp >> 32);
    const u64 q = (u64)y1 * wp1 + (((u64)y1 * wp0) >> 32) + (((u64)y0 * wp1) >> 32);
    return y * w + q * np;
#endif
}
HE_HD u64 shoup4h(u64 y, u64 w, u64 wp, u64 np) {
#if defined(__CUDA_ARCH__)
    u64 v;
    asm volatile("{\n\t"
        ".reg .u32 y0, y1, w0, w1, p0, p1, n0, n1, nh, a1, b1, q0, q1, v0, v1, z;\n\t"
        ".reg .u64 A, B, Q, V;\n\t"
        "mov.b64 {y0, y1}, %1;\n\t"
        "mov.b64 {w0, w1}, %2;\n\t"
        "mov.b64 {p0, p1}, %3;\n\t"
        "mov.b64 {n0, n1}, %4;\n\t"
        "add.u32 nh, n1, 1;\n\t"
        "mul.hi.u32 a1, y1, p0;\n\t"
        "mul.hi.u32 b1, y0, p1;\n\t"
        "mov.u32 z, 0;\n\t"
        "mov.b64 A, {a1, z};\n\t"
        "mov.b64 B, {b1, z};\n\t"
        "mad.wide.u32 Q, y1, p1, A;\n\t"
        "add.u64 Q, Q, B;\n\t"
        "mov.b64 {q0, q1}, Q;\n\t"
        "mul.wide.u32 V, y0, w0;\n\t"
        "mov.b64 {v0, v1}, V;\n\t"
        "mad.lo.u32 v1, y1, w0, v1;\n\t"
        "mad.lo.u32 v1, y0, w1, v1;\n\t"
        "mad.lo.u32 v1, q0, nh, v1;\n\t"
        "sub.cc.u32 v0, v0, q0;\n\t"
        "subc.u32 v1, v1, q1;\n\t"
        "mov.b64 %0, {v0, v1};\n\t}"
        : "=l"(v)
        : "l"(y), "l"(w), "l"(wp), "l"(np));
    return v;
#else
    const u32 y0 = (u32)y, y1 = (u32)(y >> 32), wp0 = (u32)wp, wp1 = (u32)(wp >> 32);
    const u64 q = (u64)y1 * wp1 + (((u64)y1 * wp0) >> 32) + (((u64)y0 * wp1) >> 32);
    const u64 h = (0 - np) >> 32;
    return y * w - q - ((u64)((u32)q * (u32)h) << 32);
#endif
}
template <int CLS>
HE_HD u64 shoup4c(u64 y, u64 w, u64 wp, u64 np) { return CLS == kNarrowH ? shoup4h(y, w, wp, np) : shoup4(y, w, wp, np); }
HE_HD u64 shoup2(u64 y, u64 w, u64 wp, u64 np) { return y * w + mulhi64(y, wp) * np; }

HE_HD u64 reduce_small(u64 x, const u64 p, const u64 np, const int red_shift, const u32 red_recip) {
    const u32 xs = (u32)(x >> red_shift);
    const u32 qhat = mul_hi_u32(xs, red_recip);
    u32 np0, np1, rl, rh;
    unpack64(np, np0, np1);
    unpack64(mad_wide_u32(qhat, np0, x), rl, rh);
    rh = qhat * np1 + rh;
    return csub(pack64(rl, rh), p);
}
HE_HD void reduce_small16(u64 (&x)[16], const RowMod &m) {
    const int shift = m.slot->red_shift;
    const u32 recip = m.slot->red_recip;
    const u64 p = 0 - m.np;
#pragma unroll
    for (int r = 0; r < 16; ++r) x[r] = reduce_small(x[r], p, m.np, shift, recip);
}

HE_HD u32 csub32(u32 x, u32 m) {
    const u32 d = x - m;
    return d < x ? d : x;
}
HE_HD u32 shoup32(u32 y, u32 w, u32 wp, u32 p) {
    return y * w - mul_hi_u32(y, wp) * p;
}

template <int CLS>
HE_HD void ct_butterfly(u64 &x, u64 &y, const ulonglong2 w, const RowMod &m) {
    if (CLS == kSmall) {
        const u32 p = (u32)(0 - m.np), p2 = 2 * p;
        const u32 xr = csub32((u32)x, p2);
        const u32 v = shoup32((u32)y, (u32)w.x, (u32)(w.y >> 32), p);
        x = xr + v;
        y = xr - v + p2;
    } else if (narrow_like(CLS)) {
        const u64 v = shoup4c<CLS>(y, w.x, w.y, m.np);
        const u64 xo = x + v;
        y = x - v + m.kp;
        x = xo;
    } else if (CLS == kMid) {
        const u64 xr = csub(x, m.kp);
        const u64 v = shoup4(y, w.x, w.y, m.np);
        x = xr + v;
        y = xr - v + m.kp;
    } else {
        const u64 xr = csub(x, m.kp);
        const u64 v = shoup2(y, w.x, w.y, m.np);
        x = xr + v;
        y = xr - v + m.kp;
    }
}

template <int LOGN, int LB, int C, int CLS, int J>
HE_HD void fwd_stage(u64 (&x)[16], int tau, const RowMod &m) {
    constexpr int E = pass_e(LB, C), F = 1 << E, S0 = LOGN - LB - C, T = (1 << LOGN) / 16;
    constexpr int H = 1 << (C - 1 - J);
    const int hi = tau >> (LB - E);
    const ulonglong2 *tw_t = LB == 0 ? m.tw_t() + tau : nullptr;
#pragma unroll
    for (int grp = 0; grp < (1 << J); ++grp) {
        const ulonglong2 w = LB == 0 ? ld_tw(tw_t + ((1 << J) - 1 + grp) * T)
                                     : ld_tw_cached(m, (1 << (S0 + J)) + (hi << J) + grp);
#pragma unroll
        for (int k = 0; k < H; ++k) {
            const int a = grp * 2 * H + k;
#pragma unroll
            for (int f = 0; f < F; ++f) ct_butterfly<CLS>(x[a * F + f], x[(a + H) * F + f], w, m);
        }
    }
}
template <int LOGN, int LB, int C, int CLS>
HE_HD void fwd_pass(u64 (&x)[16], int tau, const RowMod &m) {
    fwd_stage<LOGN, LB, C, CLS, 0>(x, tau, m);
    if (C > 1) fwd_stage<LOGN, LB, C, CLS, (C > 1 ? 1 : 0)>(x, tau, m);
    if (C > 2) fwd_stage<LOGN, LB, C, CLS, (C > 2 ? 2 : 0)>(x, tau, m);
    if (C > 3) fwd_stage<LOGN, LB, C, CLS, (C > 3 ? 3 : 0)>(x, tau, m);
}

template <int CLS>
HE_HD void fwd_finish(u64 (&x)[16], const RowMod &m) {
    if (CLS == kSmall) {
        const u32 p = (u32)(0 - m.np);
#pragma unroll
        for (int r = 0; r < 16; ++r) x[r] = csub32(csub32((u32)x[r], 2 * p), p);
    } else {
        reduce_small16(x, m);
    }
}

template <int CLS>
HE_HD void gs_butterfly(u64 &x, u64 &y, const ulonglong2 w, const RowMod &m, u64 kp) {
    if (CLS == kSmall) {
        const u32 p = (u32)(0 - m.np), p2 = 2 * p;
        const u32 s = csub32((u32)x + (u32)y, p2);
        y = shoup32((u32)x - (u32)y + p2, (u32)w.x, (u32)(w.y >> 32), p);
        x = s;
    } else if (narrow_like(CLS)) {
        const u64 s = x + y;
        y = shoup4c<CLS>(x - y + kp, w.x, w.y, m.np);
        x = s;
    } else if (CLS == kMid) {
        const u64 s = csub(x + y, kp);
        y = shoup4(x - y + kp, w.x, w.y, m.np);
        x = s;
    } else {
        const u64 s = csub(x + y, kp);
        y = shoup2(x - y + kp, w.x, w.y, m.np);
        x = s;
    }
}

template <int LOGN, int LB, int C, int CLS, int BIN, int J>
HE_HD void inv_stage(u64 (&x)[16], const int tau, const RowMod &m) {
    constexpr int E = pass_e(LB, C), F = 1 << E, T = (1 << LOGN) / 16;
    constexpr int HH = 1 << J;
    constexpr bool kLast = (LB + J == LOGN - 1);
    constexpr int kGroups = 1 << (LOGN - 1 - LB - J);
    const int hi = tau >> (LB - E);
    const u64 kp = narrow_like(CLS) ? (0 - m.np) * (u64)inv_bound_after(BIN, J) : m.kp;
    const ulonglong2 *tw_t = LB == 0 ? m.tw_t() + tau : nullptr;
#pragma unroll
    for (int grp = 0; grp < (1 << (C - 1 - J)); ++grp) {
        if (!kLast || m.partial) {
            const ulonglong2 w = LB == 0 ? ld_tw(tw_t + (16 - (16 >> J) + grp) * T)
                                         : ld_tw_cached(m, kGroups + (hi << (C - 1 - J)) + grp);
#pragma unroll
            for (int k = 0; k < HH; ++k) {
                const int a = grp * 2 * HH + k;
#pragma unroll
                for (int f = 0; f < F; ++f) gs_butterfly<CLS>(x[a * F + f], x[(a + HH) * F + f], w, m, kp);
            }
        } else {
            const u64 *sc = &m.slot->inv_scale[m.scale_mode].c0;
            const u64 c0 = ld_u64(sc), c0p = ld_u64(sc + 1), c1 = ld_u64(sc + 2), c1p = ld_u64(sc + 3);
#pragma unroll
            for (int k = 0; k < HH; ++k) {
                const int a = grp * 2 * HH + k;
#pragma unroll
                for (int f = 0; f < F; ++f) {
                    if (CLS == kSmall) {
                        const u32 p = (u32)(0 - m.np);
                        const u32 xa = (u32)x[a * F + f], ya = (u32)x[(a + HH) * F + f];
                        x[a * F + f] = csub32(shoup32(xa + ya, (u32)c0, (u32)(c0p >> 32), p), p);
                        x[(a + HH) * F + f] = csub32(shoup32(xa - ya + 2 * p, (u32)c1, (u32)(c1p >> 32), p), p);
                        continue;
                    }
                    const u64 xa = x[a * F + f], ya = x[(a + HH) * F + f];
                    const u64 s = xa + ya;
                    const u64 d = xa - ya + kp;
                    x[a * F + f] = csub(shoup2(s, c0, c0p, m.np), 0 - m.np);
                    x[(a + HH) * F + f] = csub(shoup2(d, c1, c1p, m.np), 0 - m.np);
                }
            }
        }
    }
}

template <int LOGN, int LB, int C, int CLS, int BIN>
HE_HD void inv_pass(u64 (&x)[16], int tau, const RowMod &m) {
    inv_stage<LOGN, LB, C, CLS, BIN, 0>(x, tau, m);
    if (C > 1) inv_stage<LOGN, LB, C, CLS, BIN, (C > 1 ? 1 : 0)>(x, tau, m);
    if (C > 2) inv_stage<LOGN, LB, C, CLS, BIN, (C > 2 ? 2 : 0)>(x, tau, m);
    if (C > 3) inv_stage<LOGN, LB, C, CLS, BIN, (C > 3 ? 3 : 0)>(x, tau, m);
}

HE_HD void inv_reduce(u64 (&x)[16], const RowMod &m) { reduce_small16(x, m); }

HE_HD int fwd_last_source(int logn, int k, int tau) {
    int j = 0;
    while ((2 << j) - 1 <= k) ++j;
    const int grp = k - ((1 << j) - 1);
    return (1 << (logn - 4 + j)) + (tau << j) + grp;
}
HE_HD int inv_first_source(int logn, int k, int tau) {
    int J = 0;
    while (16 - (16 >> (J + 1)) <= k) ++J;
    const int grp = k - (16 - (16 >> J));
    return (1 << (logn - 1 - J)) + (tau << (3 - J)) + grp;
}

}
}
```

Baseline: 158,900.

## Enable special-form auxiliary primes with cheaper Montgomery reduction across BEHZ and NTT

Auxiliary BEHZ primes are now always chosen of the form p ≡ 1 mod 2^32; this used to need an environment variable and a compile flag. A specialised Montgomery reduction for these primes uses 32-bit multiplies instead of a full 64-bit low product with ninv. The lift, tensor, floor, fused NTT-tensor and row-NTT kernels are templated on this property. The NTT kernels also get a compile-time class set, so launches where every row is narrow only instantiate the narrow paths, which cuts branching and code size. In exchange there are more kernel instantiations, and the prime selection changes for every context that uses the fast path.

```diff
diff --git a/swift-homomorphic-encryption_b200/csrc/behz.cu b/swift-homomorphic-encryption_b200/csrc/behz.cu
--- a/swift-homomorphic-encryption_b200/csrc/behz.cu
+++ b/swift-homomorphic-encryption_b200/csrc/behz.cu
@@ -1,6 +1,7 @@
 #include <cstdlib>
 
 #include "kernels.cuh"
+#include "ntt_fast.cuh"
 
 namespace hecuda {
 
@@ -36,7 +37,7 @@
     else *p = v[0];
 }
 
-template <int L, int COLS>
+template <int L, int COLS, bool H>
 __global__ void __launch_bounds__(kThreads) lift_kernel(const u64 *__restrict__ in, int polys_in, u64 *__restrict__ ext,
                                                        int ext_polys, int out_poly_offset,
                                                        const __grid_constant__ LiftConsts c, int n, bool q_rows) {
@@ -78,7 +79,7 @@
             u128 acc = (u128)rc * c.qr[j];
 #pragma unroll
             for (int i = 0; i < L; ++i) mac128(acc, z[k][i], c.mat[j][i]);
-            const u64 red = mont_reduce(acc, c.b[j], c.b_ninv[j]);
+            const u64 red = mont_reduce_c<H>(acc, c.b[j], c.b_ninv[j]);
             o[k] = c.wide_sums ? barrett64(red, c.b[j], c.b_mu1[j]) : csub(red, c.b[j]);
         }
         stc<COLS>(dst + (int64_t)(aux0 + j) * n, o);
@@ -88,9 +89,24 @@
 struct TensorConsts {
     int R;
     u64 p[kMaxRows], ninv[kMaxRows];
+    unsigned char h[kMaxRows];
 };
 
-template <int COLS>
+template <int COLS, bool H>
+__device__ __forceinline__ void tensor_cols(const Cols<COLS> &a0, const Cols<COLS> &a1, const Cols<COLS> &b0,
+                                            const Cols<COLS> &b1, u64 p, u64 ninv, u64 (&o0)[COLS], u64 (&o1)[COLS],
+                                            u64 (&o2)[COLS]) {
+#pragma unroll
+    for (int k = 0; k < COLS; ++k) {
+        o0[k] = csub(mont_reduce_c<H>((u128)a0.v[k] * b0.v[k], p, ninv), p);
+        u128 m = (u128)a0.v[k] * b1.v[k];
+        mac128(m, a1.v[k], b0.v[k]);
+        o1[k] = csub(mont_reduce_c<H>(m, p, ninv), p);
+        o2[k] = csub(mont_reduce_c<H>((u128)a1.v[k] * b1.v[k], p, ninv), p);
+    }
+}
+
+template <int COLS, bool ANY_H>
 __global__ void __launch_bounds__(kThreads) tensor_kernel(const u64 *__restrict__ ext, u64 *__restrict__ ten,
                                                          const __grid_constant__ TensorConsts c, int n) {
     const int R = c.R;
@@ -104,14 +120,8 @@
     const Cols<COLS> a0 = ldc<COLS>(e), a1 = ldc<COLS>(e + ps), b0 = ldc<COLS>(e + 2 * ps), b1 = ldc<COLS>(e + 3 * ps);
     u64 *o = ten + (item * 3 * R + row) * n + coeff;
     u64 o0[COLS], o1[COLS], o2[COLS];
-#pragma unroll
-    for (int k = 0; k < COLS; ++k) {
-        o0[k] = csub(mont_reduce((u128)a0.v[k] * b0.v[k], p, ninv), p);
-        u128 m = (u128)a0.v[k] * b1.v[k];
-        mac128(m, a1.v[k], b0.v[k]);
-        o1[k] = csub(mont_reduce(m, p, ninv), p);
-        o2[k] = csub(mont_reduce((u128)a1.v[k] * b1.v[k], p, ninv), p);
-    }
+    if (ANY_H && c.h[row]) tensor_cols<COLS, true>(a0, a1, b0, b1, p, ninv, o0, o1, o2);
+    else tensor_cols<COLS, false>(a0, a1, b0, b1, p, ninv, o0, o1, o2);
     stc<COLS>(o, o0);
     stc<COLS>(o + ps, o1);
     stc<COLS>(o + 2 * ps, o2);
@@ -171,7 +181,7 @@
     stc<2>(o + 2 * ps, o2);
 }
 
-template <int L, int COLS>
+template <int L, int COLS, bool H>
 __global__ void __launch_bounds__(kThreads) floor_kernel(const u64 *__restrict__ in, u64 *__restrict__ out,
                                                         const __grid_constant__ FloorConsts c, int n) {
     constexpr int R = 2 * L + 1;
@@ -196,7 +206,7 @@
             u128 acc = (u128)xb.v[k] * c.fq[j];
 #pragma unroll
             for (int i = 0; i < L; ++i) mac128(acc, y[k][i], c.fmat[j][i]);
-            f[k][j] = mont_reduce(acc, c.b[j], c.b_ninv[j]);
+            f[k][j] = mont_reduce_c<H>(acc, c.b[j], c.b_ninv[j]);
         }
     }
     const u64 msk = c.b[L];
@@ -210,7 +220,7 @@
             w[i] = shoup_mul(f[k][i], c.inb_w[i], c.inb_wp[i], c.b[i]);
             mac128(acc, w[i], c.amat[i]);
         }
-        u64 alpha = mont_reduce(acc, msk, c.b_ninv[L]);
+        u64 alpha = mont_reduce_c<H>(acc, msk, c.b_ninv[L]);
         alpha = c.wide_sums ? barrett64(alpha, msk, c.msk_mu1) : csub(csub(csub(alpha, 4 * msk), 2 * msk), msk);
         const bool exceeds = alpha > (msk >> 1);
         const u64 alpha_c = exceeds ? msk - alpha : alpha;
@@ -309,6 +319,20 @@
         default: return cudaErrorInvalidValue;                                                                        \
     }
 
+template <int COLS, bool H>
+static cudaError_t launch_lift_kernel(int L, dim3 grid, cudaStream_t stream, const u64 *in, int polys_in, u64 *ext,
+                                      int ext_polys, int out_poly_offset, const LiftConsts &consts, int n, bool q_rows) {
+    HE_DISPATCH_L(L, (lift_kernel<LL, COLS, H><<<grid, kThreads, 0, stream>>>(in, polys_in, ext, ext_polys, out_poly_offset,
+                                                                              consts, n, q_rows)));
+    return cudaSuccess;
+}
+template <int COLS, bool H>
+static cudaError_t launch_floor_kernel(int L, dim3 grid, cudaStream_t stream, const u64 *in, u64 *out,
+                                       const FloorConsts &consts, int n) {
+    HE_DISPATCH_L(L, (floor_kernel<LL, COLS, H><<<grid, kThreads, 0, stream>>>(in, out, consts, n)));
+    return cudaSuccess;
+}
+
 static inline dim3 poly_grid(int64_t n, int64_t polys, int cols) {
     const unsigned gx = (unsigned)((n / cols + kThreads - 1) / kThreads);
     const int64_t gy = polys < 32768 ? polys : 32768;
@@ -328,12 +352,11 @@
         ++g_kernel_launches;
         if (ctx.L > 16) {
             lift_generic_kernel<<<grid, kThreads, 0, stream>>>(in, polys_in, ext, ext_polys, out_poly_offset, consts, (int)ctx.n, q_rows);
-        } else if (cols == 2) {
-            HE_DISPATCH_L(ctx.L, (lift_kernel<LL, 2><<<grid, kThreads, 0, stream>>>(in, polys_in, ext, ext_polys,
-                                                                                 out_poly_offset, consts, (int)ctx.n, q_rows)));
         } else {
-            HE_DISPATCH_L(ctx.L, (lift_kernel<LL, 1><<<grid, kThreads, 0, stream>>>(in, polys_in, ext, ext_polys,
-                                                                                 out_poly_offset, consts, (int)ctx.n, q_rows)));
+            auto launch = cols == 2 ? (consts.h_primes ? launch_lift_kernel<2, true> : launch_lift_kernel<2, false>)
+                                    : (consts.h_primes ? launch_lift_kernel<1, true> : launch_lift_kernel<1, false>);
+            const cudaError_t e = launch(ctx.L, grid, stream, in, polys_in, ext, ext_polys, out_poly_offset, consts, (int)ctx.n, q_rows);
+            if (e != cudaSuccess) return e;
         }
         in += slab * pstride_in;
         ext += (slab / polys_in) * (int64_t)ext_polys * (q_rows ? 2 * ctx.L + 1 : ctx.L + 1) * ctx.n;
@@ -351,19 +374,18 @@
     for (int r = 0; r < tc.R; ++r) {
         tc.p[r] = ctx.slots[map.slot[r]].dev.p;
         tc.ninv[r] = ctx.slots[map.slot[r]].dev.ninv;
+        tc.h[r] = fast::class_of_modulus(tc.p[r], ctx.slots[map.slot[r]].dev.bits) == fast::kNarrowH ? 1 : 0;
     }
     const int cols = ctx.n >= 2 ? cols_per_thread() : 1;
+    bool any_h = false;
+    for (int r = 0; r < tc.R; ++r) any_h |= tc.h[r] != 0;
+    auto k = cols == 2 ? (any_h ? tensor_kernel<2, true> : tensor_kernel<2, false>) : (any_h ? tensor_kernel<1, true> : tensor_kernel<1, false>);
     const unsigned gx = (unsigned)((ctx.n / cols + kThreads - 1) / kThreads);
     for (int64_t done = 0; done < items;) {
         const int64_t chunk = (items - done) > 65535 ? 65535 : (items - done);
         dim3 grid(gx ? gx : 1, (unsigned)tc.R, (unsigned)chunk);
         ++g_kernel_launches;
-        if (cols == 2)
-            tensor_kernel<2><<<grid, kThreads, 0, stream>>>(ext + done * 4 * tc.R * ctx.n, ten + done * 3 * tc.R * ctx.n, tc,
-                                                            (int)ctx.n);
-        else
-            tensor_kernel<1><<<grid, kThreads, 0, stream>>>(ext + done * 4 * tc.R * ctx.n, ten + done * 3 * tc.R * ctx.n, tc,
-                                                            (int)ctx.n);
+        k<<<grid, kThreads, 0, stream>>>(ext + done * 4 * tc.R * ctx.n, ten + done * 3 * tc.R * ctx.n, tc, (int)ctx.n);
         done += chunk;
     }
     return cudaGetLastError();
@@ -413,10 +435,11 @@
         ++g_kernel_launches;
         if (ctx.L > 16) {
             floor_generic_kernel<<<grid, kThreads, 0, stream>>>(in, out, consts, (int)ctx.n);
-        } else if (cols == 2) {
-            HE_DISPATCH_L(ctx.L, (floor_kernel<LL, 2><<<grid, kThreads, 0, stream>>>(in, out, consts, (int)ctx.n)));
         } else {
-            HE_DISPATCH_L(ctx.L, (floor_kernel<LL, 1><<<grid, kThreads, 0, stream>>>(in, out, consts, (int)ctx.n)));
+            auto launch = cols == 2 ? (consts.h_primes ? launch_floor_kernel<2, true> : launch_floor_kernel<2, false>)
+                                    : (consts.h_primes ? launch_floor_kernel<1, true> : launch_floor_kernel<1, false>);
+            const cudaError_t e = launch(ctx.L, grid, stream, in, out, consts, (int)ctx.n);
+            if (e != cudaSuccess) return e;
         }
         in += slab * (int64_t)R * ctx.n;
         out += slab * (int64_t)ctx.L * ctx.n;
diff --git a/swift-homomorphic-encryption_b200/csrc/context.cu b/swift-homomorphic-encryption_b200/csrc/context.cu
--- a/swift-homomorphic-encryption_b200/csrc/context.cu
+++ b/swift-homomorphic-encryption_b200/csrc/context.cu
@@ -139,9 +139,8 @@
         for (u64 v : c->q) log_q += std::log2((double)v);
         const double log_n = (double)c->logn, log_t = std::log2((double)t);
         for (int wi = 0; wi < 2 && want_fast && c->aux == c->bsk && word_bits == 64; ++wi) {
-            const bool h_primes = fast::kNarrowHEnabled && std::getenv("HECUDA_AUX_H_PRIMES") != nullptr;
-            std::vector<u64> cand = (widths[wi] == 55 && h_primes) ? smallest_ntt_primes(55, L + 1 + nmod, 1ull << 31)
-                                                                   : smallest_ntt_primes(widths[wi], L + 1 + nmod, (u64)n);
+            std::vector<u64> cand = widths[wi] == 55 ? smallest_ntt_primes(55, L + 1 + nmod, 1ull << 31)
+                                                     : smallest_ntt_primes(widths[wi], L + 1 + nmod, (u64)n);
             std::vector<u64> pick;
             for (u64 v : cand) {
                 bool used = false;
@@ -244,6 +243,9 @@
     auto slot_of = [&](int j) { return reference_base ? c->slot_bsk(j) : c->slot_aux(j); };
     std::memset(&lf, 0, sizeof(lf));
     lf.L = L;
+    bool h_primes = true;
+    for (int j = 0; j <= L; ++j) h_primes &= fast::class_of_modulus(BSK[j], bit_length(BSK[j])) == fast::kNarrowH;
+    lf.h_primes = h_primes ? 1 : 0;
     {
         const u64 q_mod_mt = prod_mod(Q, L, kMTilde);
         lf.neg_inv_q_mt = (u32)((kMTilde - invmod(q_mod_mt, kMTilde)) % kMTilde);
@@ -270,6 +272,7 @@
     }
     std::memset(&fl, 0, sizeof(fl));
     fl.L = L;
+    fl.h_primes = lf.h_primes;
     const u64 b_mod_msk = prod_mod(BSK, L, msk);
     const u64 r64_msk = c->slots[slot_of(L)].dev.r64;
     const u64 b_inv_msk = mulmod(invmod(b_mod_msk, msk), r64_msk, msk);
diff --git a/swift-homomorphic-encryption_b200/csrc/context.hpp b/swift-homomorphic-encryption_b200/csrc/context.hpp
--- a/swift-homomorphic-encryption_b200/csrc/context.hpp
+++ b/swift-homomorphic-encryption_b200/csrc/context.hpp
@@ -53,6 +53,7 @@
     u64 b[kMaxL + 1], b_ninv[kMaxL + 1];
     u64 mat[kMaxL + 1][kMaxL];
     u64 qr[kMaxL + 1];
+    int h_primes;
 };
 
 struct FloorConsts {
@@ -69,6 +70,7 @@
     u64 a_msk;
     u64 omat[kMaxL][kMaxL];
     u64 b_mod_q[kMaxL], neg_b_mod_q[kMaxL];
+    int h_primes;
 };
 
 struct DivRoundConsts {
diff --git a/swift-homomorphic-encryption_b200/csrc/modarith.cuh b/swift-homomorphic-encryption_b200/csrc/modarith.cuh
--- a/swift-homomorphic-encryption_b200/csrc/modarith.cuh
+++ b/swift-homomorphic-encryption_b200/csrc/modarith.cuh
@@ -73,6 +73,14 @@
     const u64 m = lo * ninv;
     return hi + mulhi64(m, p) + (lo != 0 ? 1ull : 0ull);
 }
+HE_HD u64 mont_reduce_h(u128 acc, u64 p) {
+    const u64 lo = (u64)acc, hi = (u64)(acc >> 64);
+    const u32 h = (u32)(p >> 32), lo0 = (u32)lo, lo1 = (u32)(lo >> 32);
+    const u32 m0 = 0u - lo0, m1 = lo0 * h - lo1 - (lo0 != 0 ? 1u : 0u);
+    return hi + (u64)m1 * h + (((u64)m0 * h + m1) >> 32) + (lo != 0 ? 1ull : 0ull);
+}
+template <bool H>
+HE_HD u64 mont_reduce_c(u128 acc, u64 p, u64 ninv) { return H ? mont_reduce_h(acc, p) : mont_reduce(acc, p, ninv); }
 
 HE_HD u64 barrett_prod(u128w x, u64 p, u64 mu, int s) {
     u64 xs = (x.lo >> s) | (x.hi << (64 - s));
diff --git a/swift-homomorphic-encryption_b200/csrc/ntt_fast.cu b/swift-homomorphic-encryption_b200/csrc/ntt_fast.cu
--- a/swift-homomorphic-encryption_b200/csrc/ntt_fast.cu
+++ b/swift-homomorphic-encryption_b200/csrc/ntt_fast.cu
@@ -121,6 +121,23 @@
     inv_row_pass<LOGN, CLS, P - 1>(x, sm, tau, m);
 }
 
+template <int LOGN, unsigned CLASSES>
+__device__ __forceinline__ void fwd_row_of(int cls, u64 *sm, int tau, const RowMod &m, bool reduce_in) {
+    if (has_class(CLASSES, kNarrowH) && cls == kNarrowH) fwd_row<LOGN, kNarrowH>(sm, tau, m, reduce_in);
+    else if (has_class(CLASSES, kNarrow) && narrow_like(cls)) fwd_row<LOGN, kNarrow>(sm, tau, m, reduce_in);
+    else if (has_class(CLASSES, kSmall) && cls == kSmall) fwd_row<LOGN, kSmall>(sm, tau, m, reduce_in);
+    else if (has_class(CLASSES, kMid) && cls == kMid) fwd_row<LOGN, kMid>(sm, tau, m, reduce_in);
+    else if (has_class(CLASSES, kWide)) fwd_row<LOGN, kWide>(sm, tau, m, reduce_in);
+}
+template <int LOGN, unsigned CLASSES>
+__device__ __forceinline__ void inv_row_of(int cls, u64 *sm, int tau, const RowMod &m) {
+    if (has_class(CLASSES, kNarrowH) && cls == kNarrowH) inv_row<LOGN, kNarrowH>(sm, tau, m);
+    else if (has_class(CLASSES, kNarrow) && narrow_like(cls)) inv_row<LOGN, kNarrow>(sm, tau, m);
+    else if (has_class(CLASSES, kSmall) && cls == kSmall) inv_row<LOGN, kSmall>(sm, tau, m);
+    else if (has_class(CLASSES, kMid) && cls == kMid) inv_row<LOGN, kMid>(sm, tau, m);
+    else if (has_class(CLASSES, kWide)) inv_row<LOGN, kWide>(sm, tau, m);
+}
+
 HE_HD constexpr int ntt_row_buffers(int logn) { return logn == 13 ? 2 : 1; }
 
 template <int LOGN>
@@ -131,7 +148,7 @@
 
 constexpr int ntt_min_ctas(int logn) { return logn == 13 ? 1 : 1024 / ((1 << logn) / 16); }
 
-template <int LOGN, bool INVERSE>
+template <int LOGN, bool INVERSE, unsigned CLASSES>
 __global__ void __launch_bounds__((1 << LOGN) / 16, ntt_min_ctas(LOGN))
     ntt_rows_kernel(const __grid_constant__ CUtensorMap map_in, const __grid_constant__ CUtensorMap map_out,
                     const ModSlot *__restrict__ slots, const __grid_constant__ RowList rl, const int polys,
@@ -216,20 +233,8 @@
         if (debug_flags & 4) {
         } else
 #ifndef HE_EXPERIMENT_ONLY_CLASS
-        if (INVERSE) {
-            if (kNarrowHEnabled && cls == kNarrowH) inv_row<LOGN, kNarrowHEnabled ? kNarrowH : kNarrow>(sm, tau, m);
-            else if (cls == kNarrow) inv_row<LOGN, kNarrow>(sm, tau, m);
-            else if (cls == kSmall) inv_row<LOGN, kSmall>(sm, tau, m);
-            else if (cls == kMid) inv_row<LOGN, kMid>(sm, tau, m);
-            else inv_row<LOGN, kWide>(sm, tau, m);
-        } else {
-            const bool reduce_in = (flags & 8) != 0;
-            if (kNarrowHEnabled && cls == kNarrowH) fwd_row<LOGN, kNarrowHEnabled ? kNarrowH : kNarrow>(sm, tau, m, reduce_in);
-            else if (cls == kNarrow) fwd_row<LOGN, kNarrow>(sm, tau, m, reduce_in);
-            else if (cls == kSmall) fwd_row<LOGN, kSmall>(sm, tau, m, reduce_in);
-            else if (cls == kMid) fwd_row<LOGN, kMid>(sm, tau, m, reduce_in);
-            else fwd_row<LOGN, kWide>(sm, tau, m, reduce_in);
-        }
+        if (INVERSE) inv_row_of<LOGN, CLASSES>(cls, sm, tau, m);
+        else fwd_row_of<LOGN, CLASSES>(cls, sm, tau, m, (flags & 8) != 0);
 #else
         if (INVERSE) inv_row<LOGN, HE_EXPERIMENT_ONLY_CLASS>(sm, tau, m);
         else fwd_row<LOGN, HE_EXPERIMENT_ONLY_CLASS>(sm, tau, m, (flags & 8) != 0);
@@ -275,21 +280,46 @@
     asm volatile("ld.shared::cluster.v2.u64 {%0, %1}, [%2];" : "=l"(v.x), "=l"(v.y) : "r"(addr) : "memory");
     return v;
 }
-__device__ __forceinline__ u64 mont_product(u64 a, u64 b, u64 p, u64 ninv) { return csub(mont_reduce((u128)a * b, p, ninv), p); }
+template <bool H>
+__device__ __forceinline__ u64 mont_product(u64 a, u64 b, u64 p, u64 ninv) { return csub(mont_reduce_c<H>((u128)a * b, p, ninv), p); }
 
 template <int LOGN>
 constexpr size_t ntt_tensor_smem_bytes() {
     return sizeof(u64) * 2 * ((size_t)1 << LOGN) + sizeof(ulonglong2) * ((size_t)1 << (LOGN - 4)) + sizeof(u64) * 3;
 }
 
-template <int LOGN>
+template <int LOGN, bool H>
+__device__ __forceinline__ void tensor_step(const u64 *x, const u64 *y, u64 *out, int64_t comp, u32 rank, int tau, u64 p, u64 ninv) {
+    constexpr int N = 1 << LOGN, T = N / 16;
+    u64 *own = out + (rank ? 2 * comp : 0);
+#pragma unroll 4
+    for (int w = 2 * tau; w < N; w += 2 * T) {
+        const ulonglong2 a = *reinterpret_cast<const ulonglong2 *>(x + w), b = *reinterpret_cast<const ulonglong2 *>(y + w);
+        *reinterpret_cast<ulonglong2 *>(own + smem_phys(w)) =
+            make_ulonglong2(mont_product<H>(a.x, b.x, p, ninv), mont_product<H>(a.y, b.y, p, ninv));
+    }
+    cluster_wait();
+    const u32 px = cluster_map(smem_u32(x), rank ^ 1), py = cluster_map(smem_u32(y), rank ^ 1);
+#pragma unroll 4
+    for (int w = (int)rank * (N / 2) + 2 * tau; w < ((int)rank + 1) * (N / 2); w += 2 * T) {
+        const ulonglong2 a = *reinterpret_cast<const ulonglong2 *>(x + w), b = *reinterpret_cast<const ulonglong2 *>(y + w);
+        const ulonglong2 A = ld_cluster_v2(px + 8u * w), Bv = ld_cluster_v2(py + 8u * w);
+        u128 m0 = (u128)a.x * Bv.x, m1 = (u128)a.y * Bv.y;
+        mac128(m0, A.x, b.x);
+        mac128(m1, A.y, b.y);
+        *reinterpret_cast<ulonglong2 *>(out + comp + smem_phys(w)) =
+            make_ulonglong2(csub(mont_reduce_c<H>(m0, p, ninv), p), csub(mont_reduce_c<H>(m1, p, ninv), p));
+    }
+}
+
+template <int LOGN, unsigned CLASSES>
 __global__ void __launch_bounds__((1 << LOGN) / 16, 1)
     ntt_forward_tensor_kernel(const __grid_constant__ CUtensorMap map_lhs, const __grid_constant__ CUtensorMap map_rhs,
                               const __grid_constant__ CUtensorMap map_ext, u64 *__restrict__ ten,
                               const ModSlot *__restrict__ slots, const __grid_constant__ RowList rl, const int items,
                               const int L) {
     extern __shared__ __align__(1024) u64 smem[];
-    constexpr int N = 1 << LOGN, T = N / 16;
+    constexpr int N = 1 << LOGN;
     constexpr int kBoxes = N / kLineWords / kBoxLines;
     constexpr u32 kRowBytes = (u32)sizeof(u64) << LOGN, kTwBytes = (u32)sizeof(ulonglong2) << (LOGN - 4);
     static_assert(kBoxes >= 1, "one row is at least one box");
@@ -358,38 +388,15 @@
 #pragma unroll
         for (int j = 0; j < 2; ++j) {
             mbar_wait(&bar_row[j], phase_row);
-            u64 *sm = smem + j * N;
-            if (kNarrowHEnabled && cls == kNarrowH) fwd_row<LOGN, kNarrowHEnabled ? kNarrowH : kNarrow>(sm, tau, m, false);
-            else if (cls == kNarrow) fwd_row<LOGN, kNarrow>(sm, tau, m, false);
-            else if (cls == kSmall) fwd_row<LOGN, kSmall>(sm, tau, m, false);
-            else if (cls == kMid) fwd_row<LOGN, kMid>(sm, tau, m, false);
-            else fwd_row<LOGN, kWide>(sm, tau, m, false);
+            fwd_row_of<LOGN, CLASSES>(cls, smem + j * N, tau, m, false);
         }
         phase_row ^= 1;
         __syncthreads();
         cluster_arrive();
-        const u64 p = S.p, ninv = S.ninv;
-        const u64 *x = smem, *y = smem + N;
         const int64_t comp = (int64_t)R * N;
         u64 *out = ten + ((int64_t)3 * item * R + r) * N;
-        u64 *own = out + (rank ? 2 * comp : 0);
-#pragma unroll 4
-        for (int w = 2 * tau; w < N; w += 2 * T) {
-            const ulonglong2 a = *reinterpret_cast<const ulonglong2 *>(x + w), b = *reinterpret_cast<const ulonglong2 *>(y + w);
-            *reinterpret_cast<ulonglong2 *>(own + smem_phys(w)) = make_ulonglong2(mont_product(a.x, b.x, p, ninv), mont_product(a.y, b.y, p, ninv));
-        }
-        cluster_wait();
-        const u32 px = cluster_map(smem_u32(x), rank ^ 1), py = cluster_map(smem_u32(y), rank ^ 1);
-#pragma unroll 4
-        for (int w = (int)rank * (N / 2) + 2 * tau; w < ((int)rank + 1) * (N / 2); w += 2 * T) {
-            const ulonglong2 a = *reinterpret_cast<const ulonglong2 *>(x + w), b = *reinterpret_cast<const ulonglong2 *>(y + w);
-            const ulonglong2 A = ld_cluster_v2(px + 8u * w), Bv = ld_cluster_v2(py + 8u * w);
-            u128 m0 = (u128)a.x * Bv.x, m1 = (u128)a.y * Bv.y;
-            mac128(m0, A.x, b.x);
-            mac128(m1, A.y, b.y);
-            *reinterpret_cast<ulonglong2 *>(out + comp + smem_phys(w)) =
-                make_ulonglong2(csub(mont_reduce(m0, p, ninv), p), csub(mont_reduce(m1, p, ninv), p));
-        }
+        if (has_class(CLASSES, kNarrowH) && cls == kNarrowH) tensor_step<LOGN, true>(smem, smem + N, out, comp, rank, tau, S.p, S.ninv);
+        else tensor_step<LOGN, false>(smem, smem + N, out, comp, rank, tau, S.p, S.ninv);
         fence_proxy_async_smem();
         cluster_arrive_relaxed();
     }
@@ -447,21 +454,24 @@
                CU_TENSOR_MAP_FLOAT_OOB_FILL_NONE) == CUDA_SUCCESS;
 }
 
-template <int LOGN, bool INVERSE>
-static cudaError_t launch_logn(const Context &ctx, const NttRowMap &map, const u64 *in, u64 *out, int64_t rows,
+static bool narrow_h_rows(const RowList &rl) {
+    bool any_h = false;
+    for (int i = 0; i < rl.count; ++i) {
+        const int cls = rl.flags[i] & 7;
+        if (!narrow_like(cls)) return false;
+        any_h |= cls == kNarrowH;
+    }
+    return any_h;
+}
+
+template <int LOGN, bool INVERSE, unsigned CLASSES>
+static cudaError_t launch_rows(const Context &ctx, const RowList &rl, const u64 *in, u64 *out, int polys, int64_t rows,
                                int scale_mode, cudaStream_t stream) {
-    if (rows % map.rows_per_poly) return cudaErrorInvalidValue;
-    if (rows == 0) return cudaSuccess;
-    if (rows > 0x7fffffffLL) return cudaErrorInvalidValue;
-    RowList rl;
-    build_row_list(ctx, map, INVERSE, rl);
-    if (rl.src_poly_stride % kLineWords) return cudaErrorInvalidValue;
     CUtensorMap map_in, map_out;
     if (!make_line_map(&map_in, in, LOGN) || !make_line_map(&map_out, out, LOGN)) return cudaErrorInvalidValue;
-    const int polys = (int)(rows / map.rows_per_poly);
     constexpr int threads = (1 << LOGN) / 16;
     constexpr size_t smem = ntt_smem_bytes<LOGN>();
-    auto k = ntt_rows_kernel<LOGN, INVERSE>;
+    auto k = ntt_rows_kernel<LOGN, INVERSE, CLASSES>;
     static int ctas_per_sm[64] = {0};
     static std::mutex mu;
     int per_sm;
@@ -486,6 +496,21 @@
     }();
     k<<<(unsigned)grid, threads, smem, stream>>>(map_in, map_out, ctx.d_slots, rl, polys, scale_mode, debug_flags);
     return cudaGetLastError();
+}
+
+template <int LOGN, bool INVERSE>
+static cudaError_t launch_logn(const Context &ctx, const NttRowMap &map, const u64 *in, u64 *out, int64_t rows,
+                               int scale_mode, cudaStream_t stream) {
+    if (rows % map.rows_per_poly) return cudaErrorInvalidValue;
+    if (rows == 0) return cudaSuccess;
+    if (rows > 0x7fffffffLL) return cudaErrorInvalidValue;
+    RowList rl;
+    build_row_list(ctx, map, INVERSE, rl);
+    if (rl.src_poly_stride % kLineWords) return cudaErrorInvalidValue;
+    const int polys = (int)(rows / map.rows_per_poly);
+    if (LOGN == 13 && narrow_h_rows(rl))
+        return launch_rows<LOGN, INVERSE, (LOGN == 13 ? kNarrowClasses : kAllClasses)>(ctx, rl, in, out, polys, rows, scale_mode, stream);
+    return launch_rows<LOGN, INVERSE, kAllClasses>(ctx, rl, in, out, polys, rows, scale_mode, stream);
 }
 
 struct SplitRows {
@@ -580,7 +605,7 @@
     {
         constexpr int threads = (1 << LOGN) / 16;
         constexpr size_t smem = ntt_smem_bytes<LOGN>();
-        auto k = ntt_rows_kernel<LOGN, INVERSE>;
+        auto k = ntt_rows_kernel<LOGN, INVERSE, kAllClasses>;
         cudaError_t e;
         if ((e = cudaFuncSetAttribute(k, cudaFuncAttributeMaxDynamicSharedMemorySize, (int)smem)) != cudaSuccess) return e;
         int per_sm = 0;
@@ -624,20 +649,16 @@
     return launch_fast<true>(ctx, map, in, out, rows, scale_mode, stream);
 }
 
-cudaError_t launch_ntt_forward_tensor(const Context &ctx, const NttRowMap &map, const u64 *lhs, const u64 *rhs,
-                                      const u64 *ext, u64 *ten, int64_t items, cudaStream_t stream) {
+template <unsigned CLASSES>
+static cudaError_t launch_forward_tensor(const Context &ctx, const RowList &rl, const u64 *lhs, const u64 *rhs,
+                                         const u64 *ext, u64 *ten, int64_t items, cudaStream_t stream) {
     constexpr int LOGN = 13;
-    if (ctx.logn != LOGN) return cudaErrorInvalidValue;
-    if (items == 0) return cudaSuccess;
-    if (items * 4 * map.rows_per_poly * (ctx.n / kLineWords) > 0x7fffffffLL) return cudaErrorInvalidValue;
-    RowList rl;
-    build_row_list(ctx, map, false, rl);
     CUtensorMap map_lhs, map_rhs, map_ext;
     if (!make_line_map(&map_lhs, lhs, LOGN) || !make_line_map(&map_rhs, rhs, LOGN) || !make_line_map(&map_ext, ext, LOGN))
         return cudaErrorInvalidValue;
     constexpr int threads = (1 << LOGN) / 16;
     constexpr size_t smem = ntt_tensor_smem_bytes<LOGN>();
-    auto k = ntt_forward_tensor_kernel<LOGN>;
+    auto k = ntt_forward_tensor_kernel<LOGN, CLASSES>;
     cudaLaunchAttribute attr[1];
     attr[0].id = cudaLaunchAttributeClusterDimension;
     attr[0].val.clusterDim.x = 2;
@@ -673,4 +694,15 @@
     return e != cudaSuccess ? e : cudaGetLastError();
 }
 
-}
+cudaError_t launch_ntt_forward_tensor(const Context &ctx, const NttRowMap &map, const u64 *lhs, const u64 *rhs,
+                                      const u64 *ext, u64 *ten, int64_t items, cudaStream_t stream) {
+    if (ctx.logn != 13) return cudaErrorInvalidValue;
+    if (items == 0) return cudaSuccess;
+    if (items * 4 * map.rows_per_poly * (ctx.n / kLineWords) > 0x7fffffffLL) return cudaErrorInvalidValue;
+    RowList rl;
+    build_row_list(ctx, map, false, rl);
+    if (narrow_h_rows(rl)) return launch_forward_tensor<kNarrowClasses>(ctx, rl, lhs, rhs, ext, ten, items, stream);
+    return launch_forward_tensor<kAllClasses>(ctx, rl, lhs, rhs, ext, ten, items, stream);
+}
+
+}
diff --git a/swift-homomorphic-encryption_b200/csrc/ntt_fast.cuh b/swift-homomorphic-encryption_b200/csrc/ntt_fast.cuh
--- a/swift-homomorphic-encryption_b200/csrc/ntt_fast.cuh
+++ b/swift-homomorphic-encryption_b200/csrc/ntt_fast.cuh
@@ -14,15 +14,15 @@
 HE_HD constexpr int class_of_bits(int bits) {
     return bits <= kSmallBits ? kSmall : bits <= kNarrowBits ? kNarrow : bits <= kMidBits ? kMid : kWide;
 }
-#if defined(HE_NTT_NARROW_H)
-constexpr bool kNarrowHEnabled = true;
-#else
-constexpr bool kNarrowHEnabled = false;
-#endif
 HE_HD constexpr int class_of_modulus(u64 p, int bits) {
-    return (kNarrowHEnabled && class_of_bits(bits) == kNarrow && (u32)p == 1u) ? kNarrowH : class_of_bits(bits);
+    return (class_of_bits(bits) == kNarrow && (u32)p == 1u) ? kNarrowH : class_of_bits(bits);
 }
 HE_HD constexpr bool narrow_like(int cls) { return cls == kNarrow || cls == kNarrowH; }
+
+HE_HD constexpr unsigned class_bit(int cls) { return 1u << cls; }
+constexpr unsigned kAllClasses = (1u << kNarrow) | (1u << kMid) | (1u << kWide) | (1u << kSmall);
+constexpr unsigned kNarrowClasses = (1u << kNarrow) | (1u << kNarrowH);
+HE_HD constexpr bool has_class(unsigned set, int cls) { return (set & class_bit(cls)) != 0; }
 
 HE_HD constexpr int plan_passes(int logn) { return logn <= 12 ? 3 : 4; }
 HE_HD constexpr int plan_c(int logn, int k) {
```

Result: faster. 165,500, median of 6 (+4.2%).
